# Yelp/nrtsearch

Hardware: AMD Instinct MI355X
Metric: queries/sec, 10M-doc 5-term BM25 top-1000 (higher is better)
Workload: dtype f32

## Files before the change

include/nrtgpu_dev.h:

```cpp
#ifndef NRTGPU_DEV_H
#define NRTGPU_DEV_H
#include "nrtgpu.h"
#ifdef __cplusplus
extern "C" {
#endif
int  nrtgpu_bench_closed_loop(nrtgpu_ctx* ctx, const nrtgpu_seg* const* segs, const int32_t* doc_bases, int32_t n_segs,
                              const nrtgpu_bm25_query* queries, int32_t n_queries, int32_t clients, int32_t duration_ms,
                              double* out4);
int  nrtgpu_debug_hold_coalescers(nrtgpu_ctx* ctx, int32_t hold);
int  nrtgpu_debug_coalescer_pending(nrtgpu_ctx* ctx, int32_t which);
int  nrtgpu_debug_dist_inject(nrtgpu_ctx* ctx, int32_t step, int32_t failed_query);
int64_t nrtgpu_debug_live_segments(nrtgpu_ctx* ctx);
int  nrtgpu_debug_spec_counters(nrtgpu_ctx* ctx, int64_t* out3);
int  nrtgpu_debug_term_lookup(const nrtgpu_seg* seg, int32_t field_id, int64_t term_hash, int32_t* kind, int32_t* shift, int64_t* bytes);
int  nrtgpu_debug_knn_bounds(int32_t sim, int32_t dim, double q_norm2, double q_l1, float q_absmax, double nv_max, double nv_min,
                             float rows_absmax, float score_boost, double m, double s, double* out10);
int  nrtgpu_debug_knn_unpack(const float* scores, const int32_t* docs, const uint32_t* counts, int32_t k_stride, int32_t n_queries,
                             int32_t k_pass, const int32_t* ks, const float* boosts, nrtgpu_topdocs* out);

#define NRTGPU_FLAG_PROFILE (7 << 8)
int  nrtgpu_get_scan_profile(nrtgpu_ctx* ctx, double* out16);
int  nrtgpu_get_maxscore_profile(nrtgpu_ctx* ctx, double* out16);
int  nrtgpu_debug_maxscore_meetings(nrtgpu_ctx* ctx, int64_t* out4);
int  nrtgpu_debug_maxscore_meeting_guesses(nrtgpu_ctx* ctx, int64_t* out1);
int  nrtgpu_debug_wave_kth(const uint64_t* keys, int32_t n, int32_t r, uint64_t* out);
int64_t nrtgpu_debug_walk_rows(nrtgpu_ctx* ctx, const nrtgpu_seg* const* segs, const int32_t* doc_bases, int32_t n_segs,
                               const nrtgpu_bm25_query* queries, int32_t n_queries, int32_t* out_begin, int32_t* out_n,
                               uint64_t* out_rows, int64_t cap_rows);
int  nrtgpu_debug_walk_value(float weight, const uint32_t* freq, const uint32_t* norm, int32_t n, const float* table256, int32_t fx_scale,
                             uint32_t fx_shift, uint64_t* out);
int64_t nrtgpu_get_maxscore_item_walls(nrtgpu_ctx* ctx, uint64_t* out, int64_t cap_slots, int64_t* n_items);

#ifdef __cplusplus
}
#endif
#endif
```

nrtsearch_amd/_lib.py:

```python
from __future__ import annotations

import ctypes as C
import os

_HERE = os.path.dirname(os.path.abspath(__file__))
LIB_PATH = os.environ.get("NRTGPU_LIB_PATH") or os.path.join(_HERE, "libnrtgpu.so")

NRTGPU_OK = 0
NRTGPU_ERR_INVALID_ARG = -1
NRTGPU_ERR_HIP = -2
NRTGPU_ERR_OOM = -3
NRTGPU_ERR_UNSUPPORTED = -4
NRTGPU_ERR_STATE = -5
NRTGPU_ERR_TIMEOUT = -6
NRTGPU_MAX_K = 1024
NRTGPU_MAX_TERMS = 32
NRTGPU_TILE_DOCS = 1024
NRTGPU_FLAG_NO_PREFETCH = 1
NRTGPU_FLAG_NO_FIXED_POINT = 2
NRTGPU_FLAG_NO_MASK_VARIANT = 4
NRTGPU_FLAG_NO_LIVE_FOLD = 8
NRTGPU_FLAG_NO_PRUNE = 16
NRTGPU_FLAG_PACKED_POSTINGS = 32
NRTGPU_FLAG_BLOCKING_WAIT = 64
NRTGPU_FLAG_NO_VECTOR_SKETCH = 128
NRTGPU_FLAG_PROFILE = 7 << 8
NRTGPU_MAX_MASKS = 8
NRTGPU_MAX_FUNCTIONS = 8
NRTGPU_MAX_GROUPS = 8
NRTGPU_GROUPS_SUM_OF_MAX = 0
NRTGPU_GROUPS_MAX_OF_SUM = 1
NRTGPU_MAX_KNN_LISTS = 8
NRTGPU_DOCVALUES_INT32 = 0
NRTGPU_DOCVALUES_FLOAT32 = 1
NRTGPU_MAX_TERM_BUCKETS = 65536

ABI_SYMBOLS = [
    "nrtgpu_version", "nrtgpu_last_error", "nrtgpu_create", "nrtgpu_destroy",
    "nrtgpu_segment_begin", "nrtgpu_segment_add_field_norms", "nrtgpu_segment_add_terms",
    "nrtgpu_segment_add_vectors", "nrtgpu_segment_seal", "nrtgpu_segment_set_live_docs",
    "nrtgpu_segment_set_mask", "nrtgpu_segment_release", "nrtgpu_segment_device_bytes",
    "nrtgpu_search_bm25", "nrtgpu_search_bm25_batch", "nrtgpu_search_bm25_batch_device",
    "nrtgpu_search_bm25_batch_device_epoch", "nrtgpu_exchange_open", "nrtgpu_exchange_close",
    "nrtgpu_search_bm25_coalesced", "nrtgpu_set_coalescing", "nrtgpu_query_supported",
    "nrtgpu_merge_topk_device", "nrtgpu_knn_exact", "nrtgpu_knn_exact_coalesced", "nrtgpu_knn_search", "nrtgpu_knn_search_requests", "nrtgpu_knn_search_coalesced", "nrtgpu_rescore_vectors", "nrtgpu_search_hybrid_batch",
    "nrtgpu_int_to_byte4", "nrtgpu_byte4_to_int", "nrtgpu_bm25_idf", "nrtgpu_bm25_avgdl",
    "nrtgpu_bm25_norm_cache", "nrtgpu_slices", "nrtgpu_plan_item_counts", "nrtgpu_fixed_point_scale", "nrtgpu_get_stats", "nrtgpu_reset_stats",
    "nrtgpu_set_slicing",
    "nrtgpu_blend", "nrtgpu_dist_unique_id", "nrtgpu_dist_init", "nrtgpu_dist_search_bm25_batch", "nrtgpu_dist_allgather_merge", "nrtgpu_segment_fork",
    "nrtgpu_search_bm25_batch_device_begin", "nrtgpu_pending_wait", "nrtgpu_set_thread_deadline_ns", "nrtgpu_monotonic_ns", "nrtgpu_last_diagnostics", "nrtgpu_dist_close", "nrtgpu_dist_owned_range", "nrtgpu_dist_search_bm25_batch_mode", "nrtgpu_dist_exchange_merge", "nrtgpu_dist_exchange_merge_checked", "nrtgpu_search_bm25_shard_device_begin", "nrtgpu_note_shard_speculation", "nrtgpu_dist_knn_exact", "nrtgpu_dist_search_hybrid_batch",
    "nrtgpu_knn_exact_relation", "nrtgpu_set_speculation", "nrtgpu_set_shard_share", "nrtgpu_set_thread_slices",
    "nrtgpu_segment_add_byte_vectors", "nrtgpu_knn_exact_bytes", "nrtgpu_knn_search_bytes", "nrtgpu_byte_vector_score",
    "nrtgpu_knn_search_bytes_requests", "nrtgpu_knn_search_bytes_coalesced", "nrtgpu_knn_exact_bytes_coalesced",
    "nrtgpu_rescore_byte_vectors", "nrtgpu_search_hybrid_bytes_batch", "nrtgpu_set_knn_gather",
    "nrtgpu_search_function_score_batch", "nrtgpu_function_score_supported", "nrtgpu_function_score_value",
    "nrtgpu_search_multi_match_batch", "nrtgpu_multi_match_supported", "nrtgpu_multi_match_value",
    "nrtgpu_search_function_score_multi_match_batch", "nrtgpu_function_score_multi_match_supported", "nrtgpu_function_score_multi_match_value",
    "nrtgpu_search_text_knn_batch", "nrtgpu_text_knn_supported", "nrtgpu_text_knn_value", "nrtgpu_text_knn_exact",
    "nrtgpu_segment_add_doc_values", "nrtgpu_search_sorted_batch", "nrtgpu_sorted_supported", "nrtgpu_sort_value_code",
    "nrtgpu_count_terms_batch", "nrtgpu_count_terms_supported",
]
DEV_SYMBOLS = [
    "nrtgpu_bench_closed_loop", "nrtgpu_debug_hold_coalescers", "nrtgpu_debug_coalescer_pending", "nrtgpu_debug_live_segments",
    "nrtgpu_debug_spec_counters", "nrtgpu_get_scan_profile", "nrtgpu_get_maxscore_profile", "nrtgpu_get_maxscore_item_walls",
    "nrtgpu_debug_dist_inject", "nrtgpu_debug_term_lookup", "nrtgpu_debug_knn_bounds", "nrtgpu_debug_knn_unpack",
    "nrtgpu_debug_maxscore_meetings", "nrtgpu_debug_wave_kth", "nrtgpu_debug_walk_rows", "nrtgpu_debug_walk_value",
    "nrtgpu_debug_maxscore_meeting_guesses",
]
DEV_LIB_PATH = os.path.join(_HERE, "libnrtgpu_dev.so")


class Config(C.Structure):
    _fields_ = [("device_id", C.c_int32), ("max_batch", C.c_int32), ("target_items", C.c_int32),
                ("collect_timing", C.c_int32), ("flags", C.c_int32), ("host_threads", C.c_int32),
                ("lookup_budget_pct", C.c_int32), ("reserved", C.c_int32)]


class Term(C.Structure):
    _fields_ = [("field_id", C.c_int32), ("cache_slot", C.c_int32), ("term_hash", C.c_int64),
                ("weight", C.c_float), ("occur", C.c_int32)]


class Bm25Query(C.Structure):
    _fields_ = [("n_terms", C.c_int32), ("terms", C.POINTER(Term)), ("n_caches", C.c_int32),
                ("norm_cache", C.POINTER(C.c_float)), ("k", C.c_int32), ("total_hits_threshold", C.c_int32),
                ("has_after", C.c_int32), ("after_doc", C.c_int32), ("after_score", C.c_float),
                ("min_should_match", C.c_int32), ("min_competitive_score", C.c_float), ("filter_mask", C.c_int32),
                ("must_not_mask", C.c_int32), ("disjunction_max", C.c_int32),
                ("n_more_filters", C.c_int32), ("more_filters", C.POINTER(C.c_int32)),
                ("n_more_must_not", C.c_int32), ("more_must_not", C.POINTER(C.c_int32)),
                ("tie_breaker", C.c_float), ("reserved", C.c_int32)]


class ScoreFunction(C.Structure):
    _fields_ = [("filter_mask", C.c_int32), ("weight", C.c_float)]


class FunctionScore(C.Structure):
    _fields_ = [("n_functions", C.c_int32), ("functions", C.POINTER(ScoreFunction)), ("score_mode", C.c_int32),
                ("boost_mode", C.c_int32), ("min_score", C.c_float), ("min_excluded", C.c_int32)]


class ClauseGroups(C.Structure):
    _fields_ = [("shape", C.c_int32), ("n_groups", C.c_int32), ("group_of_term", C.POINTER(C.c_int32)),
                ("group_min_should_match", C.POINTER(C.c_int32)), ("tie_breaker", C.c_float), ("group_occur", C.c_int32)]


class DocScores(C.Structure):
    _fields_ = [("docs", C.POINTER(C.c_int32)), ("scores", C.POINTER(C.c_float)), ("n", C.c_int32), ("boost", C.c_float)]


class KnnClauses(C.Structure):
    _fields_ = [("lists", C.POINTER(DocScores)), ("n_lists", C.c_int32), ("text_nested", C.c_int32)]


class TopDocs(C.Structure):
    _fields_ = [("n_hits", C.c_int32), ("capacity", C.c_int32), ("docs", C.POINTER(C.c_int32)),
                ("scores", C.POINTER(C.c_float)), ("total_hits", C.c_int64),
                ("total_hits_is_lower_bound", C.c_int32)]


class FieldSort(C.Structure):
    _fields_ = [("field_id", C.c_int32), ("reverse", C.c_int32), ("missing_bits", C.c_uint32), ("has_after", C.c_int32),
                ("after_doc", C.c_int32), ("after_bits", C.c_uint32)]


class FieldDocs(C.Structure):
    _fields_ = [("n_hits", C.c_int32), ("capacity", C.c_int32), ("docs", C.POINTER(C.c_int32)),
                ("value_bits", C.POINTER(C.c_uint32)), ("total_hits", C.c_int64),
                ("total_hits_is_lower_bound", C.c_int32)]


class TermsCount(C.Structure):
    _fields_ = [("field_id", C.c_int32), ("max_buckets", C.c_int32)]


class TermCounts(C.Structure):
    _fields_ = [("n_buckets", C.c_int32), ("capacity", C.c_int32), ("value_bits", C.POINTER(C.c_uint32)), ("counts", C.POINTER(C.c_int32)),
                ("total_hits", C.c_int64), ("hits_with_value", C.c_int64), ("overflowed", C.c_int32), ("reserved", C.c_int32)]


class Diagnostics(C.Structure):
    _fields_ = [("total_ms", C.c_double), ("plan_ms", C.c_double), ("queue_ms", C.c_double), ("device_ms", C.c_double),
                ("postings", C.c_int64), ("queries", C.c_int32), ("items_maxscore", C.c_int32), ("items_scan", C.c_int32),
                ("reserved", C.c_int32)]


class Stats(C.Structure):
    _fields_ = [("batches", C.c_int64), ("queries", C.c_int64), ("scan_launches", C.c_int64),
                ("scan_ms", C.c_double), ("scan_postings", C.c_int64), ("scan_items", C.c_int64),
# ... 65 lines not shown
    L.nrtgpu_exchange_close.restype = None
    L.nrtgpu_merge_topk_device.argtypes = [vp, i32, i32, i32, vp, vp, vp, vp, vp, C.POINTER(TopDocs)]
    L.nrtgpu_knn_exact.argtypes = [vp, vp, vp, i32, i32, i32, vp, i32, i32, i32, f32, C.POINTER(TopDocs)]
    L.nrtgpu_knn_exact_coalesced.argtypes = [vp, vp, vp, i32, i32, i32, vp, i32, i32, f32, C.POINTER(TopDocs)]
    L.nrtgpu_knn_exact_coalesced.restype = i32
    L.nrtgpu_knn_search.argtypes = [vp, vp, vp, i32, i32, i32, vp, i32, i32, i32, f32, i32, f32, C.POINTER(TopDocs)]
    L.nrtgpu_knn_search_requests.argtypes = [vp, vp, vp, i32, i32, i32, vp, i32, i32, vp, vp, vp, vp, C.POINTER(TopDocs)]
    L.nrtgpu_knn_search_coalesced.argtypes = [vp, vp, vp, i32, i32, i32, vp, i32, i32, f32, i32, f32, C.POINTER(TopDocs)]
    L.nrtgpu_knn_search_coalesced.restype = i32
    L.nrtgpu_segment_add_byte_vectors.argtypes = [vp, i32, i32, i32, vp, vp]
    L.nrtgpu_knn_exact_bytes.argtypes = [vp, vp, vp, i32, i32, i32, vp, i32, i32, i32, f32, C.POINTER(TopDocs)]
    L.nrtgpu_knn_search_bytes.argtypes = [vp, vp, vp, i32, i32, i32, vp, i32, i32, i32, f32, i32, f32, C.POINTER(TopDocs)]
    L.nrtgpu_knn_search_bytes_requests.argtypes = [vp, vp, vp, i32, i32, i32, vp, i32, i32, vp, vp, vp, vp, C.POINTER(TopDocs)]
    L.nrtgpu_knn_search_bytes_coalesced.argtypes = [vp, vp, vp, i32, i32, i32, vp, i32, i32, f32, i32, f32, C.POINTER(TopDocs)]
    L.nrtgpu_knn_search_bytes_coalesced.restype = i32
    L.nrtgpu_knn_exact_bytes_coalesced.argtypes = [vp, vp, vp, i32, i32, i32, vp, i32, i32, f32, C.POINTER(TopDocs)]
    L.nrtgpu_knn_exact_bytes_coalesced.restype = i32
    L.nrtgpu_byte_vector_score.argtypes = [i32, i32, i32, i32, i32, vp]
    L.nrtgpu_set_knn_gather.argtypes = [vp, i32]
    L.nrtgpu_search_function_score_batch.argtypes = [vp, vp, vp, i32, C.POINTER(Bm25Query), C.POINTER(FunctionScore), i32, C.POINTER(TopDocs)]
    L.nrtgpu_function_score_supported.argtypes = [vp, vp, i32, C.POINTER(Bm25Query), C.POINTER(FunctionScore)]
    L.nrtgpu_function_score_value.argtypes = [C.POINTER(FunctionScore), C.c_uint32, f32, vp, vp]
    L.nrtgpu_search_multi_match_batch.argtypes = [vp, vp, vp, i32, C.POINTER(Bm25Query), C.POINTER(ClauseGroups), i32, C.POINTER(TopDocs)]
    L.nrtgpu_multi_match_supported.argtypes = [vp, vp, i32, C.POINTER(Bm25Query), C.POINTER(ClauseGroups)]
    L.nrtgpu_multi_match_value.argtypes = [C.POINTER(ClauseGroups), i32, vp, i32, vp, C.c_uint32, vp, vp]
    L.nrtgpu_search_function_score_multi_match_batch.argtypes = [vp, vp, vp, i32, C.POINTER(Bm25Query), C.POINTER(ClauseGroups), C.POINTER(FunctionScore), i32,
                                                                 C.POINTER(TopDocs)]
    L.nrtgpu_function_score_multi_match_supported.argtypes = [vp, vp, i32, C.POINTER(Bm25Query), C.POINTER(ClauseGroups), C.POINTER(FunctionScore)]
    L.nrtgpu_function_score_multi_match_value.argtypes = [C.POINTER(ClauseGroups), i32, vp, i32, vp, C.c_uint32, C.POINTER(FunctionScore), C.c_uint32, vp, vp]
    L.nrtgpu_search_text_knn_batch.argtypes = [vp, vp, vp, i32, C.POINTER(Bm25Query), C.POINTER(KnnClauses), i32, C.POINTER(TopDocs)]
    L.nrtgpu_text_knn_supported.argtypes = [vp, vp, i32, C.POINTER(Bm25Query), C.POINTER(KnnClauses)]
    L.nrtgpu_text_knn_value.argtypes = [i32, i32, C.c_uint64, i32, C.c_double, vp]
    L.nrtgpu_text_knn_exact.argtypes = [C.POINTER(Bm25Query), C.POINTER(KnnClauses), i32]
    L.nrtgpu_segment_add_doc_values.argtypes = [vp, i32, i32, i32, vp, vp]
    L.nrtgpu_search_sorted_batch.argtypes = [vp, vp, vp, i32, C.POINTER(Bm25Query), C.POINTER(FieldSort), i32, C.POINTER(FieldDocs)]
    L.nrtgpu_sorted_supported.argtypes = [vp, vp, i32, C.POINTER(Bm25Query), C.POINTER(FieldSort)]
    L.nrtgpu_sort_value_code.argtypes = [i32, i32, C.c_uint32, vp]
    L.nrtgpu_count_terms_batch.argtypes = [vp, vp, vp, i32, C.POINTER(Bm25Query), C.POINTER(TermsCount), i32, C.POINTER(TermCounts)]
    L.nrtgpu_count_terms_supported.argtypes = [vp, vp, i32, C.POINTER(Bm25Query), C.POINTER(TermsCount)]
    L.nrtgpu_rescore_vectors.argtypes = [vp, vp, vp, i32, i32, i32, vp, i32, f32, vp, vp, i32, C.c_double, C.c_double, i32,
                                         C.POINTER(TopDocs)]
    L.nrtgpu_search_hybrid_batch.argtypes = [vp, vp, vp, i32, C.POINTER(Bm25Query), i32, i32, i32, vp, i32, f32,
                                             C.c_double, C.c_double, i32, C.POINTER(TopDocs)]
    L.nrtgpu_rescore_byte_vectors.argtypes = L.nrtgpu_rescore_vectors.argtypes
    L.nrtgpu_search_hybrid_bytes_batch.argtypes = L.nrtgpu_search_hybrid_batch.argtypes
    L.nrtgpu_int_to_byte4.argtypes = [i32]
    L.nrtgpu_byte4_to_int.argtypes = [i32]
    L.nrtgpu_bm25_idf.argtypes = [i64, i64]
    L.nrtgpu_bm25_idf.restype = f32
    L.nrtgpu_bm25_avgdl.argtypes = [i64, i64]
    L.nrtgpu_bm25_avgdl.restype = f32
    L.nrtgpu_bm25_norm_cache.argtypes = [f32, f32, f32, vp]
    L.nrtgpu_bm25_norm_cache.restype = None
    L.nrtgpu_plan_item_counts.argtypes = [i32, vp, i32, vp]
    L.nrtgpu_fixed_point_scale.argtypes = [f32, vp, i32, vp]
    L.nrtgpu_slices.argtypes = [i32, vp, vp, vp, i32, i32, i32, vp, vp]
    L.nrtgpu_get_stats.argtypes = [vp, C.POINTER(Stats)]
    L.nrtgpu_reset_stats.argtypes = [vp]
    L.nrtgpu_set_thread_slices.argtypes = [vp, i32]
    L.nrtgpu_set_speculation.argtypes = [vp, C.c_float]
    L.nrtgpu_set_speculation.restype = C.c_int
    L.nrtgpu_set_shard_share.argtypes = [vp, C.c_int64, C.c_int64]
    L.nrtgpu_set_shard_share.restype = C.c_int
    L.nrtgpu_knn_exact_relation.argtypes = [vp, vp, vp, C.c_int32, C.c_int32, C.c_int32, C.c_int32]
    L.nrtgpu_reset_stats.restype = None
    if hasattr(L, "nrtgpu_debug_hold_coalescers"):
        L.nrtgpu_debug_hold_coalescers.argtypes = [vp, C.c_int32]
        L.nrtgpu_debug_live_segments.argtypes = [vp]
        L.nrtgpu_debug_live_segments.restype = C.c_int64
        L.nrtgpu_debug_spec_counters.argtypes = [vp, vp]
        L.nrtgpu_debug_spec_counters.restype = C.c_int
        L.nrtgpu_get_maxscore_item_walls.argtypes = [vp, vp, C.c_int64, C.POINTER(C.c_int64)]
        L.nrtgpu_get_maxscore_item_walls.restype = C.c_int64
        L.nrtgpu_debug_coalescer_pending.argtypes = [vp, C.c_int32]
        L.nrtgpu_debug_dist_inject.argtypes = [vp, C.c_int32, C.c_int32]
        L.nrtgpu_get_scan_profile.argtypes = [vp, vp]
        L.nrtgpu_get_maxscore_profile.argtypes = [vp, vp]
        L.nrtgpu_debug_term_lookup.argtypes = [vp, i32, i64, C.POINTER(i32), C.POINTER(i32), C.POINTER(i64)]
    if hasattr(L, "nrtgpu_debug_maxscore_meetings"):
        L.nrtgpu_debug_maxscore_meetings.argtypes = [vp, vp]
        L.nrtgpu_debug_wave_kth.argtypes = [vp, i32, i32, vp]
    if hasattr(L, "nrtgpu_debug_maxscore_meeting_guesses"):
        L.nrtgpu_debug_maxscore_meeting_guesses.argtypes = [vp, vp]
    if hasattr(L, "nrtgpu_debug_walk_rows"):
        L.nrtgpu_debug_walk_rows.argtypes = [vp, vp, vp, i32, vp, i32, vp, vp, vp, i64]
        L.nrtgpu_debug_walk_rows.restype = C.c_int64
        L.nrtgpu_debug_walk_value.argtypes = [f32, vp, vp, i32, vp, i32, C.c_uint32, vp]
    if hasattr(L, "nrtgpu_debug_knn_bounds"):
        L.nrtgpu_debug_knn_bounds.argtypes = [i32, i32, C.c_double, C.c_double, f32, C.c_double, C.c_double, f32, f32, C.c_double, C.c_double, vp]
    if hasattr(L, "nrtgpu_debug_knn_unpack"):
        L.nrtgpu_debug_knn_unpack.argtypes = [vp, vp, vp, i32, i32, i32, vp, vp, C.POINTER(TopDocs)]
    L.nrtgpu_set_slicing.argtypes = [vp, i32, i32, i32]
    L.nrtgpu_blend.argtypes = [i32, vp, vp, vp, vp, i32, i32, i32, i32, C.POINTER(TopDocs)]
    L.nrtgpu_dist_unique_id.argtypes = [vp]
    L.nrtgpu_dist_init.argtypes = [vp, i32, i32, vp]
    L.nrtgpu_dist_search_bm25_batch.argtypes = [vp, vp, vp, i32, C.POINTER(Bm25Query), i32, C.POINTER(TopDocs)]
    L.nrtgpu_dist_allgather_merge.argtypes = [vp, i32, i32, vp, vp, vp, vp, vp, C.POINTER(TopDocs)]
    L.nrtgpu_segment_fork.argtypes = [vp, vp, i32, C.POINTER(vp)]
    L.nrtgpu_search_bm25_batch_device_begin.argtypes = [vp, vp, vp, i32, C.POINTER(Bm25Query), i32, i32, vp, vp, vp, C.c_int64, vp]
    L.nrtgpu_pending_wait.argtypes = [vp]
    L.nrtgpu_set_thread_deadline_ns.argtypes = [C.c_int64]
    L.nrtgpu_set_thread_deadline_ns.restype = None
    L.nrtgpu_monotonic_ns.argtypes = []
    L.nrtgpu_monotonic_ns.restype = C.c_int64
    L.nrtgpu_last_diagnostics.argtypes = [vp]
    L.nrtgpu_dist_owned_range.argtypes = [vp, i32, i32, vp, vp]
    L.nrtgpu_dist_search_bm25_batch_mode.argtypes = [vp, vp, vp, i32, C.POINTER(Bm25Query), i32, i32, C.POINTER(TopDocs)]
    L.nrtgpu_dist_exchange_merge.argtypes = [vp, i32, i32, vp, vp, vp, vp, vp, i32, C.POINTER(TopDocs)]
    L.nrtgpu_dist_exchange_merge_checked.argtypes = [vp, i32, i32, vp, vp, vp, vp, vp, vp, i32, C.POINTER(TopDocs), vp, vp]
    L.nrtgpu_search_bm25_shard_device_begin.argtypes = [vp, vp, vp, i32, C.POINTER(Bm25Query), i32, i32, vp, vp, vp, i32, vp, vp]
    L.nrtgpu_note_shard_speculation.argtypes = [vp, vp, i32, i32, i32]
    L.nrtgpu_dist_knn_exact.argtypes = [vp, vp, vp, i32, i32, i32, vp, i32, i32, i32, C.c_float, i32, C.POINTER(TopDocs)]
    L.nrtgpu_dist_search_hybrid_batch.argtypes = [vp, vp, vp, i32, C.POINTER(Bm25Query), i32, i32, i32, vp, i32, C.c_float, C.c_double, C.c_double,
                                                  i32, i32, C.POINTER(TopDocs)]
    L.nrtgpu_dist_close.argtypes = [vp]
    L.nrtgpu_dist_close.restype = None
    return L


def check(rc: int) -> None:
    if rc != NRTGPU_OK:
        raise NrtGpuError(rc, load().nrtgpu_last_error().decode("utf-8", "replace"))
```

nrtsearch_amd/api.py:

```python
from __future__ import annotations

import ctypes as C
import dataclasses
import os
import threading
from typing import Dict, List, Optional, Sequence, Tuple, Union

import numpy as np

from . import _lib
from ._lib import NrtGpuError

INT_MAX = 2**31 - 1
TOTAL_HITS_THRESHOLD = 1000


EXCHANGE_ALLGATHER, EXCHANGE_ALLTOALL = 0, 1
EXCHANGE_NO_SPECULATION = 0x100


@dataclasses.dataclass(frozen=True)
class TermQuery:
    field: int
    term: int
# ... 260 lines not shown
    def idf(self, doc_freq: int, doc_count: int) -> np.float32:
        return np.float32(_lib.load().nrtgpu_bm25_idf(int(doc_count), int(doc_freq)))

    def avgdl(self, cs: CollectionStatistics) -> np.float32:
        return np.float32(_lib.load().nrtgpu_bm25_avgdl(int(cs.sum_total_term_freq), int(cs.doc_count)))

    def norm_cache(self, cs: CollectionStatistics) -> np.ndarray:
        out = np.zeros(256, dtype=np.float32)
        _lib.load().nrtgpu_bm25_norm_cache(C.c_float(float(self.avgdl(cs))), C.c_float(self.k1), C.c_float(self.b),
                                          out.ctypes.data)
        return out

    def scorer(self, boost: float, cs: CollectionStatistics, doc_freq: int) -> Tuple[np.float32, np.ndarray]:
        idf = self.idf(doc_freq, cs.doc_count)
        return np.float32(np.float32(boost) * idf), self.norm_cache(cs)


class GpuContext:
    def __init__(self, device_id: int = 0, max_batch: int = 1024, target_items: int = 0,
                 collect_timing: bool = False, flags: int = 0, host_threads: int = 0, lookup_budget_pct: int = 0):
        L = _lib.load()
        if os.environ.get("NRTGPU_PACKED_POSTINGS", "") not in ("", "0"):
            flags |= _lib.NRTGPU_FLAG_PACKED_POSTINGS
        self.flags = flags
        if lookup_budget_pct == 0 and os.environ.get("NRTGPU_TEST_LOOKUP_BUDGET_PCT"):
            lookup_budget_pct = int(os.environ["NRTGPU_TEST_LOOKUP_BUDGET_PCT"])
        cfg = _lib.Config(device_id, max_batch, target_items, int(collect_timing), flags, host_threads, int(lookup_budget_pct), 0)
        h = C.c_void_p()
        _lib.check(L.nrtgpu_create(C.byref(cfg), C.byref(h)))
        self._h = h
        self.max_batch = max_batch

    def set_slicing(self, slice_max_docs: int = 250_000, slice_max_segments: int = 5, virtual_shards: int = 1) -> None:
        _lib.check(_lib.load().nrtgpu_set_slicing(self._h, int(slice_max_docs), int(slice_max_segments), int(virtual_shards)))

    @staticmethod
    def dist_unique_id() -> bytes:
        buf = C.create_string_buffer(128)
        _lib.check(_lib.load().nrtgpu_dist_unique_id(buf))
        return bytes(buf.raw)

    def dist_init(self, world: int, rank: int, unique_id: bytes) -> None:
        _lib.check(_lib.load().nrtgpu_dist_init(self._h, int(world), int(rank), C.c_char_p(unique_id)))

    def dist_close(self) -> None:
        _lib.load().nrtgpu_dist_close(self._h)

    def exchange_open(self, shm_name: str, world: int, rank: int) -> None:
        _lib.check(_lib.load().nrtgpu_exchange_open(self._h, shm_name.encode(), int(world), int(rank)))

    def exchange_close(self) -> None:
        _lib.load().nrtgpu_exchange_close(self._h)

    def stats(self) -> dict:
        st = _lib.Stats()
        _lib.check(_lib.load().nrtgpu_get_stats(self._h, C.byref(st)))
        return {n: getattr(st, n) for n, _ in _lib.Stats._fields_}

    def scan_profile(self) -> dict:
        out = np.zeros(16, dtype=np.float64)
        _lib.check(_lib.load().nrtgpu_get_scan_profile(self._h, out.ctypes.data))
        names = ["prologue_cycles", "rendezvous_wait_cycles", "rendezvous_cycles", "walk_cycles", "epilogue_cycles",
                 "rendezvous", "compactions", "subtiles", "rz_select_cycles", "sparse_subtiles", "rz_keep_cycles",
                 "rz_publish_append_cycles", "candidate_subtiles", "maybe_subtiles", "last_wave_finish_cycles",
                 "first_wave_finish_cycles"]
        return dict(zip(names, out.tolist()))

    def maxscore_profile(self) -> dict:
        out = np.zeros(16, dtype=np.float64)
        _lib.check(_lib.load().nrtgpu_get_maxscore_profile(self._h, out.ctypes.data))
        names = ["windows", "compactions", "chunks", "postings_streamed", "postings_surviving", "docs_evaluated", "lookups",
                 "candidates", "prologue_cycles", "item_cycles", "waves_meeting_cycles", "waves_idle_cycles", "waves_part_prologue_cycles",
                 "waves_walk_cycles", "last_wave_out_cycles", "epilogue_cycles"]
        return dict(zip(names, out.tolist()))

    def maxscore_meetings(self) -> dict:
        out = np.zeros(4, dtype=np.int64)
        _lib.check(_lib.load().nrtgpu_debug_maxscore_meetings(self._h, out.ctypes.data))
        res = dict(zip(["meetings", "overflow_meetings", "compactions", "wave_estimates"], (int(x) for x in out)))
        g = np.zeros(1, dtype=np.int64)
        _lib.check(_lib.load().nrtgpu_debug_maxscore_meeting_guesses(self._h, g.ctypes.data))
        res["meeting_guesses"] = int(g[0])
        return res

    @staticmethod
    def set_thread_deadline(seconds_from_now: Optional[float]) -> None:
        L = _lib.load()
        L.nrtgpu_set_thread_deadline_ns(0 if seconds_from_now is None else int(L.nrtgpu_monotonic_ns() + seconds_from_now * 1e9))

    @staticmethod
    def last_diagnostics() -> dict:
        d = _lib.Diagnostics()
        _lib.check(_lib.load().nrtgpu_last_diagnostics(C.byref(d)))
        return {n: getattr(d, n) for n, _ in _lib.Diagnostics._fields_ if n != "reserved"}

    def reset_stats(self) -> None:
        _lib.load().nrtgpu_reset_stats(self._h)

    def maxscore_item_walls(self):
        L = _lib.load()
        n_items = C.c_int64(0)
        n = int(L.nrtgpu_get_maxscore_item_walls(self._h, None, 0, C.byref(n_items)))
        out = np.zeros((max(n, 0), 8), dtype=np.uint64)
        if n > 0:
            L.nrtgpu_get_maxscore_item_walls(self._h, out.ctypes.data, n, C.byref(n_items))
        return out, int(n_items.value)

    @staticmethod
    def set_thread_slices(slice_of_leaf: Optional[Sequence[int]]) -> None:
        if slice_of_leaf is None:
            _lib.check(_lib.load().nrtgpu_set_thread_slices(None, 0))
        else:
            a = np.ascontiguousarray(slice_of_leaf, dtype=np.int32)
            _lib.check(_lib.load().nrtgpu_set_thread_slices(a.ctypes.data, len(a)))

    def set_speculation(self, margin: float) -> None:
        _lib.check(_lib.load().nrtgpu_set_speculation(self._h, C.c_float(float(margin))))

    def set_knn_gather(self, max_accept_permille: int) -> None:
        _lib.check(_lib.load().nrtgpu_set_knn_gather(self._h, int(max_accept_permille)))

    def set_shard_share(self, shard_docs: int, index_docs: int) -> None:
        _lib.check(_lib.load().nrtgpu_set_shard_share(self._h, int(shard_docs), int(index_docs)))

    def spec_counters(self) -> dict:
        st = self.stats()
        return {"queries": int(st["spec_queries"]), "reruns": int(st["spec_reruns"]), "switched_off": bool(st["spec_disabled"]),
                "scattered": bool(st["spec_scattered"])}

    def debug_live_segments(self) -> int:
        return int(_lib.load().nrtgpu_debug_live_segments(self._h))

    def debug_hold_coalescers(self, hold: bool) -> None:
        _lib.check(_lib.load().nrtgpu_debug_hold_coalescers(self._h, 1 if hold else 0))

    def debug_coalescer_pending(self, which: int) -> int:
        return int(_lib.load().nrtgpu_debug_coalescer_pending(self._h, int(which)))

    def debug_dist_inject(self, step: int = -1, failed_query: int = -1) -> None:
        _lib.check(_lib.load().nrtgpu_debug_dist_inject(self._h, int(step), int(failed_query)))

    def close(self) -> None:
        if getattr(self, "_h", None):
            _lib.load().nrtgpu_destroy(self._h)
            self._h = None

    def __del__(self):
        try:
            self.close()
        except Exception:
            pass


class GpuSegment:

    def __init__(self, ctx: GpuContext, max_doc: int, doc_base: int = 0):
        self.ctx, self.max_doc, self.doc_base = ctx, int(max_doc), int(doc_base)
        h = C.c_void_p()
        _lib.check(_lib.load().nrtgpu_segment_begin(ctx._h, self.max_doc, 0, C.byref(h)))
        self._h = h

    @classmethod
    def from_data(cls, ctx: GpuContext, seg, field: int = 0, omit_norms: bool = False,
                  omit_freqs: bool = False) -> "GpuSegment":
        g = cls(ctx, seg.max_doc, seg.doc_base)
        g.add_field_norms(field, None if omit_norms else seg.norms)
# ... 852 lines not shown
```

nrtsearch_amd/csrc/devtools.cpp:

```cpp
#include "runtime_internal.h"
#include "../../include/nrtgpu_dev.h"

extern "C" int nrtgpu_bench_closed_loop(nrtgpu_ctx* ctx, const nrtgpu_seg* const* segs, const int32_t* doc_bases,
                                        int32_t n_segs, const nrtgpu_bm25_query* queries, int32_t n_queries,
                                        int32_t clients, int32_t duration_ms, double* out4) {
  if (!ctx || !queries || !out4 || n_queries <= 0 || clients <= 0 || duration_ms <= 0)
    return fail(NRTGPU_ERR_INVALID_ARG, "bad closed-loop arguments");
  std::vector<std::vector<float>> lat((size_t)clients);
  std::vector<int> rcs((size_t)clients, 0);
  std::vector<std::string> errs((size_t)clients);
  const auto t_begin = std::chrono::steady_clock::now();
  const auto t_stop = t_begin + std::chrono::milliseconds(duration_ms);
  auto client = [&](int c) {
    int32_t kmax = 1;
    for (int i = 0; i < n_queries; ++i) kmax = std::max(kmax, queries[i].k);
    std::vector<int32_t> docs((size_t)kmax);
    std::vector<float> scores((size_t)kmax);
    size_t i = (size_t)c * 7919u;
    for (;;) {
      const auto t0 = std::chrono::steady_clock::now();
      if (t0 >= t_stop) break;
      nrtgpu_topdocs o{};
      o.capacity = kmax;
      o.docs = docs.data();
      o.scores = scores.data();
      const int rc = nrtgpu_search_bm25_coalesced(ctx, segs, doc_bases, n_segs, &queries[i % (size_t)n_queries], &o);
      if (rc != 0) {
        rcs[(size_t)c] = rc;
        errs[(size_t)c] = g_last_error;
        break;
      }
      lat[(size_t)c].push_back(std::chrono::duration<float, std::milli>(std::chrono::steady_clock::now() - t0).count());
      ++i;
    }
  };
  std::vector<std::thread> pool;
  for (int c = 0; c < clients; ++c) pool.emplace_back(client, c);
  for (auto& t : pool) t.join();
  const double secs = std::chrono::duration<double>(std::chrono::steady_clock::now() - t_begin).count();
  for (int c = 0; c < clients; ++c)
    if (rcs[(size_t)c] != 0) return fail(rcs[(size_t)c], "client %d: %s", c, errs[(size_t)c].c_str());
  std::vector<float> all;
  for (auto& v : lat) all.insert(all.end(), v.begin(), v.end());
  std::sort(all.begin(), all.end());
  out4[0] = (double)all.size();
  out4[1] = secs;
  out4[2] = all.empty() ? 0.0 : all[all.size() / 2];
  out4[3] = all.empty() ? 0.0 : all[(size_t)((double)all.size() * 0.99)];
  return NRTGPU_OK;
}


extern "C" int nrtgpu_debug_knn_bounds(int32_t sim, int32_t dim, double q_norm2, double q_l1, float q_absmax, double nv_max, double nv_min,
                                       float rows_absmax, float score_boost, double m, double s, double* out10) {
  if (!out10 || sim < 0 || sim > 3 || dim <= 0 || (dim & 15)) return fail(NRTGPU_ERR_INVALID_ARG, "bad knn_bounds arguments");
  float q_scale = 1.0f, rows_scale = 1.0f;
  const bool q_ok = hostmath::knn_sketch_scale(q_absmax, &q_scale), rows_ok = hostmath::knn_sketch_scale(rows_absmax, &rows_scale);
  const double e_rel = (double)hostmath::knn_e_rel(), b = (double)score_boost;
  const float e32 = hostmath::knn_bound32(sim, dim, q_norm2, nv_max, b);
  const float e16 = hostmath::knn_bound16(sim, dim, q_norm2, q_l1, 1.0 / (double)q_scale, nv_max, nv_min, 1.0 / (double)rows_scale, b);
  out10[0] = (double)e32;
  out10[1] = (double)e16;
  out10[2] = knn_result_upper(sim, m, (double)e32, e_rel, b);
  out10[3] = knn_result_upper(sim, m, (double)e16, e_rel, b);
  out10[4] = knn_estimate_lower(sim, s, (double)e32, e_rel, b);
  out10[5] = knn_estimate_lower(sim, s, (double)e16, e_rel, b);
  out10[6] = (double)q_scale;
  out10[7] = (double)rows_scale;
  out10[8] = q_ok ? 1.0 : 0.0;
  out10[9] = rows_ok ? 1.0 : 0.0;
  return NRTGPU_OK;
}

extern "C" int nrtgpu_debug_knn_unpack(const float* scores, const int32_t* docs, const uint32_t* counts, int32_t k_stride, int32_t n_queries,
                                       int32_t k_pass, const int32_t* ks, const float* boosts, nrtgpu_topdocs* out) {
  if (!scores || !docs || !counts || !out || n_queries <= 0 || k_pass <= 0 || k_stride < k_pass) return fail(NRTGPU_ERR_INVALID_ARG, "bad knn_unpack arguments");
  std::vector<uint64_t> keys((size_t)n_queries * (size_t)k_stride, 0ull);
  for (size_t i = 0; i < keys.size(); ++i)
    if ((uint32_t)(i % (size_t)k_stride) < counts[i / (size_t)k_stride]) keys[i] = pack_key(scores[i], (uint32_t)docs[i]);
  const KnnUniform one{k_pass, 0, 1.0f, 0.0f};
  std::vector<int32_t> k_of((size_t)n_queries, k_pass);
  std::vector<float> boost_of((size_t)n_queries, 1.0f);
  const KnnAsk each{ks ? ks : k_of.data(), boosts ? boosts : boost_of.data(), nullptr, nullptr, 1};
  knn_unpack_topdocs(keys.data(), counts, (uint32_t)k_stride, n_queries, false, 0, true, ks || boosts ? each : one.ask(), out);
  return NRTGPU_OK;
}

extern "C" int nrtgpu_debug_knn_query_stats(const float* queries, int32_t n_queries, int32_t dim, float* norm2, float* max_abs, double* l1,
                                            float* ref_norm2) {
  if (!queries || !norm2 || !max_abs || !l1 || !ref_norm2 || n_queries <= 0 || dim <= 0) return fail(NRTGPU_ERR_INVALID_ARG, "bad knn_query_stats arguments");
  knn_query_stats(queries, n_queries, dim, norm2, max_abs, l1);
  for (int32_t q = 0; q < n_queries; ++q) ref_norm2[q] = float_qnorm2(queries + (size_t)q * dim, dim);
  return NRTGPU_OK;
}

extern "C" int nrtgpu_debug_maxscore_meetings(nrtgpu_ctx* ctx, int64_t* out4) {
  if (!ctx || !out4) return fail(NRTGPU_ERR_INVALID_ARG, "NULL argument");
  std::lock_guard<std::mutex> lk(ctx->stats_mu);
  for (int i = 0; i < 4; ++i) out4[i] = ctx->ms_meetings[i];
  return NRTGPU_OK;
}

extern "C" int nrtgpu_debug_maxscore_meeting_guesses(nrtgpu_ctx* ctx, int64_t* out1) {
  if (!ctx || !out1) return fail(NRTGPU_ERR_INVALID_ARG, "NULL argument");
  std::lock_guard<std::mutex> lk(ctx->stats_mu);
  *out1 = ctx->ms_meetings[4];
  return NRTGPU_OK;
}

extern "C" int nrtgpu_debug_wave_kth(const uint64_t* keys, int32_t n, int32_t r, uint64_t* out) {
  if (!keys || !out || n < 1 || n > kMsCandCap || r < 1 || r > n) return fail(NRTGPU_ERR_INVALID_ARG, "bad wave_kth arguments (1 <= r <= n <= %d)", kMsCandCap);
  uint64_t* d = nullptr;
  if (hipMalloc((void**)&d, ((size_t)n + 1) * sizeof(uint64_t)) != hipSuccess) return fail(NRTGPU_ERR_OOM, "hipMalloc");
  hipError_t e = hipMemcpy(d, keys, (size_t)n * sizeof(uint64_t), hipMemcpyHostToDevice);
  if (e == hipSuccess) {
    launch_debug_wave_kth(nullptr, d, (uint32_t)n, (uint32_t)r, d + n);
    e = hipGetLastError();
  }
  if (e == hipSuccess) e = hipMemcpy(out, d + n, sizeof(uint64_t), hipMemcpyDeviceToHost);
  (void)hipFree(d);
  if (e != hipSuccess) return fail(NRTGPU_ERR_HIP, "wave_kth: %s", hipGetErrorString(e));
  return NRTGPU_OK;
}

extern "C" int64_t nrtgpu_debug_walk_rows(nrtgpu_ctx* ctx, const nrtgpu_seg* const* segs, const int32_t* doc_bases, int32_t n_segs,
                                          const nrtgpu_bm25_query* queries, int32_t n_queries, int32_t* out_begin, int32_t* out_n,
                                          uint64_t* out_rows, int64_t cap_rows) {
  if (!ctx || !segs || !queries || !out_begin || !out_n || (!out_rows && cap_rows > 0)) return -(int64_t)fail(NRTGPU_ERR_INVALID_ARG, "NULL argument");
  if (n_queries <= 0 || n_segs <= 0 || cap_rows < 0) return -(int64_t)fail(NRTGPU_ERR_INVALID_ARG, "n_queries and n_segs must be > 0");
  if (hipSetDevice(ctx->device) != hipSuccess) return -(int64_t)fail(NRTGPU_ERR_HIP, "hipSetDevice");
  for (int si = 0; si < n_segs; ++si)
    if (!segs[si]) return -(int64_t)fail(NRTGPU_ERR_INVALID_ARG, "segment %d is NULL", si);
  SegReadLocks content(segs, n_segs);
  HostPlan hp;
  if (int rc = build_plan(ctx, segs, doc_bases, n_segs, queries, n_queries, hp, 1)) return -(int64_t)rc;
  const size_t n_pairs = (size_t)n_queries * (size_t)n_segs;
  for (size_t i = 0; i < n_pairs; ++i) out_begin[i] = -1, out_n[i] = 0;
  if (hp.n_dterms == 0) return 0;
  Carver c;
  const size_t o_qx = c.take(sizeof(DExpandHead) + hp.qexpand.size() * sizeof(DQExpand)) + sizeof(DExpandHead), o_qt = c.take(hp.qterms.size() * sizeof(DQTerm));
  const size_t o_qsb = c.take(hp.qs_begin.size() * 4), o_caches = c.take(hp.caches.size() * sizeof(float));
  const size_t o_queries = c.take(hp.queries.size() * sizeof(DQuery)), o_up = c.off;
  const size_t o_terms = c.take((size_t)hp.n_dterms * sizeof(DTerm)), o_rows = c.take((size_t)hp.n_dterms * sizeof(DWalkRow));
  std::vector<char> hb(c.off, 0);
  memcpy(hb.data() + o_qx, hp.qexpand.data(), hp.qexpand.size() * sizeof(DQExpand));
  if (!hp.qterms.empty()) memcpy(hb.data() + o_qt, hp.qterms.data(), hp.qterms.size() * sizeof(DQTerm));
  memcpy(hb.data() + o_qsb, hp.qs_begin.data(), hp.qs_begin.size() * 4);
  if (!hp.caches.empty()) memcpy(hb.data() + o_caches, hp.caches.data(), hp.caches.size() * sizeof(float));
  memcpy(hb.data() + o_queries, hp.queries.data(), hp.queries.size() * sizeof(DQuery));
  char* db = nullptr;
  if (hipMalloc((void**)&db, c.off) != hipSuccess) return -(int64_t)fail(NRTGPU_ERR_OOM, "hipMalloc");
  DExpandHead xh{};
  xh.caches = (const float*)(db + o_caches);
  xh.queries = (const DQuery*)(db + o_queries);
  xh.rows = (DWalkRow*)(db + o_rows);
  memcpy(hb.data() + o_qx - sizeof(DExpandHead), &xh, sizeof(xh));
  hipError_t e = hipMemcpy(db, hb.data(), o_up, hipMemcpyHostToDevice);
  if (e == hipSuccess) e = hipMemset(db + o_up, 0, c.off - o_up);
  if (e == hipSuccess) {
    launch_expand_terms(nullptr, (const DQExpand*)(db + o_qx), (const DQTerm*)(db + o_qt), (const uint32_t*)(db + o_qsb), (uint32_t)n_queries,
                        hp.n_leaves, (DTerm*)(db + o_terms));
    e = hipGetLastError();
  }
  if (e == hipSuccess) e = hipMemcpy(hb.data() + o_rows, db + o_rows, (size_t)hp.n_dterms * sizeof(DWalkRow), hipMemcpyDeviceToHost);
  (void)hipFree(db);
  if (e != hipSuccess) return -(int64_t)fail(NRTGPU_ERR_HIP, "walk_rows: %s", hipGetErrorString(e));
  static_assert(sizeof(DWalkRow) == 80, "ten words per row");
  if (out_rows) memcpy(out_rows, hb.data() + o_rows, (size_t)std::min<int64_t>(cap_rows, (int64_t)hp.n_dterms) * sizeof(DWalkRow));
  std::vector<uint32_t> begins;
  for (size_t i = 0; i < n_pairs; ++i)
    if (hp.qs_begin[i] != 0xFFFFFFFFu) begins.push_back(hp.qs_begin[i]);
  std::sort(begins.begin(), begins.end());
  for (size_t i = 0; i < n_pairs; ++i) {
    const uint32_t b = hp.qs_begin[i];
    if (b == 0xFFFFFFFFu || hp.qexpand[i / (size_t)n_segs].by_weight == 0u) continue;
    auto nx = std::upper_bound(begins.begin(), begins.end(), b);
    out_begin[i] = (int32_t)b;
    out_n[i] = (int32_t)((nx == begins.end() ? hp.n_dterms : *nx) - b);
  }
  return (int64_t)hp.n_dterms;
}

extern "C" int nrtgpu_debug_walk_value(float weight, const uint32_t* freq, const uint32_t* norm, int32_t n, const float* table256, int32_t fx_scale,
                                       uint32_t fx_shift, uint64_t* out) {
  if (!freq || !norm || !table256 || !out || n < 1 || fx_shift > 31u) return fail(NRTGPU_ERR_INVALID_ARG, "bad walk_value arguments");
// ... 17 lines not shown
```

nrtsearch_amd/csrc/maxscore.hip:

```cpp
#include <hip/hip_runtime.h>
#include <stdint.h>

#include <type_traits>

#include "bm25_common.hiph"

namespace nrtgpu {

constexpr int kMsWinWords = kMsWinDocs / 32;
constexpr int kSl = kMsSlots;
typedef uint32_t u32x2 __attribute__((ext_vector_type(2)));
typedef const NRT_GLOBAL u32x2* gvec2_ptr;

struct alignas(16) WClause {
  uint64_t docids, fnorm;
  uint64_t begin;
  uint32_t count, pad0;
  float    weight;
  int32_t  fx_scale;
  uint32_t flags;
  uint32_t pad;
  uint64_t u_after;
  uint64_t look;
  uint64_t cells, start;
// ... 150 lines not shown
      const uint64_t pb = exchange_bound(*xch, query, q2_hi != 0u ? (uint64_t)q2_hi << 32 : 0ull, tid);
      if (tid == 0 && pb > s.theta) {
        s.theta = pb;
        s.thr = acc_threshold<true>(pb, fx_E);
        atomicMax(theta_g, (unsigned long long)pb);
      }
    }
  } else {
    if (r != 0u && cnt0 > r) guess = topk_kth_union<kMsThreads>(s.cand, cnt0, r, &s.sc, [](auto&&) {}, 0u);
    if (tid == 0) s.cnt = cnt0;
  }
  if (tid == 0 && s.spec_z16 != 0u) {
    if (guess > s.theta) {
      s.theta = guess;
      s.thr = acc_threshold<true>(guess, fx_E);
      atomicMax(theta_g, (unsigned long long)guess);
      atomicMax(s.spec_slot, (unsigned long long)guess);
      s.n_est += 0x10000u;
    }
    const uint32_t ws = s.wins_started;
    s.spec_at = ws >= s.q_wins ? 0u : max(ws * s.spec_grow16 / 16u, ws + (uint32_t)kMsWaves);
  }
  __syncthreads();
  if (tid == 0) s.rz_flag = 0;
  __syncthreads();
}

__device__ __forceinline__ bool ms_meet(MsSmem& s, uint32_t k, int fx_E, unsigned long long* theta_g, const DExchange* xch = nullptr,
                                        uint32_t query = 0) {
  __syncthreads();
  if (!__hip_atomic_load(&s.rz_flag, __ATOMIC_RELAXED, __HIP_MEMORY_SCOPE_WORKGROUP)) return false;
  ms_compact((__attribute__((address_space(3))) MsSmem*)&s, k, fx_E, theta_g, xch, query);
  return true;
}

__device__ __noinline__ void ms_estimate(__attribute__((address_space(3))) MsSmem* sp, uint32_t k, int fx_E,
                                         unsigned long long* theta_g, const DExchange* xch) {
  MsSmem& s = *(MsSmem*)sp;
  const uint32_t lane = threadIdx.x & 63u;
  const uint32_t ws = (uint32_t)__builtin_amdgcn_readfirstlane((int)__hip_atomic_load(&s.wins_started, __ATOMIC_RELAXED, __HIP_MEMORY_SCOPE_WORKGROUP));
  const uint32_t at = (uint32_t)__builtin_amdgcn_readfirstlane((int)__hip_atomic_load(&s.spec_at, __ATOMIC_RELAXED, __HIP_MEMORY_SCOPE_WORKGROUP));
  const uint32_t n = (uint32_t)__builtin_amdgcn_readfirstlane((int)__hip_atomic_load(&s.cnt, __ATOMIC_RELAXED, __HIP_MEMORY_SCOPE_WORKGROUP));
  if (at != 0u && ws >= at && n <= (uint32_t)kMsCandCap) {
    const bool exchanging = xch && xch->world > 1u;
    uint32_t r = 0;
    if (s.spec_z16 != 0u && !exchanging && __hip_atomic_load(&s.prune_on, __ATOMIC_RELAXED, __HIP_MEMORY_SCOPE_WORKGROUP) != 0u) {
      const float m = (float)k * fminf(1.0f, (float)ws / (float)max(s.q_wins, 1u));
      const float rr = m + (float)s.spec_z16 * (1.0f / 16.0f) * sqrtf(m) + 2.0f;
      r = rr < (float)k ? (uint32_t)rr : 0u;
    }
    uint64_t guess = 0;
    if (r != 0u && n > r) guess = topk_kth_wave(s.cand, n, r, &s.sc);
    if (lane == 0u) {
      if (guess > s.theta) {
        __hip_atomic_store(&s.theta, guess, __ATOMIC_RELAXED, __HIP_MEMORY_SCOPE_WORKGROUP);
        __hip_atomic_store(&s.thr, acc_threshold<true>(guess, fx_E), __ATOMIC_RELAXED, __HIP_MEMORY_SCOPE_WORKGROUP);
        atomicMax(theta_g, (unsigned long long)guess);
        atomicMax(s.spec_slot, (unsigned long long)guess);
      }
      s.spec_at = ws >= s.q_wins ? 0u : max(ws * s.spec_grow16 / 16u, ws + (uint32_t)kMsWaves);
      s.n_est += 1u;
    }
  }
  wave_lds_phase();
  if (lane == 0u) __hip_atomic_store(&s.spec_busy, 0u, __ATOMIC_RELEASE, __HIP_MEMORY_SCOPE_WORKGROUP);
}

__device__ __forceinline__ bool ms_reserve(MsSmem& s, uint32_t lane, uint32_t mine, uint32_t& pos) {
  const uint32_t incl = scan64_dpp(mine);
  const uint32_t wave_total = (uint32_t)__builtin_amdgcn_readlane((int)incl, 63);
  uint32_t wbase = 0;
  if (lane == 0) {
    wbase = atomicAdd(&s.cnt, wave_total);
    if (wbase + wave_total > (uint32_t)kMsCandCap) {
      if (wbase <= (uint32_t)kMsCandCap) s.cnt_valid = wbase;
      __hip_atomic_store(&s.rz_flag, 1u, __ATOMIC_RELAXED, __HIP_MEMORY_SCOPE_WORKGROUP);
    }
  }
  wbase = (uint32_t)__builtin_amdgcn_readfirstlane((int)wbase);
  pos = wbase + incl - mine;
  return wbase + wave_total <= (uint32_t)kMsCandCap;
}

template <bool PROF, bool PACKED, int SHAPES>
__global__ __launch_bounds__(kMsThreads)
void bm25_maxscore_kernel(const MsArgs* __restrict__ launch) {
  constexpr bool TWO = SHAPES == 2;
  constexpr bool kMsHalfBody = kSl == 8;
  __shared__ MsSmem s;
  const uint32_t tid = threadIdx.x;
  const uint32_t wave = tid >> 6, lane = tid & 63u;
  for (uint32_t round = 0;; ++round) {
    const uint64_t wall_entry = PROF ? wall_clock64() : 0ull;
    const ms_args_ptr ap = ms_fresh(launch);
    const __attribute__((address_space(4))) DHelp& hp = ap->help;
    const DItem* const items = as_global(ap->items);
    const DPart* const parts = as_global(ap->parts);
    const DWalkRow* const rows = as_global(ap->rows);
  #ifdef NRTGPU_DEV
    const DTerm* const terms = as_global(ap->terms);
  #endif
    const DExchange* const xch = as_global(ap->xch);
    bool helper = false;
    uint32_t my_item = 0, out_slot = 0;
    {
      const uint32_t min_rem = hp.min_rem & 0xFFFFu;
      const bool greedy = ((hp.min_rem >> 16) & 1u) != 0u;
      for (int attempt = 0; attempt < 2; ++attempt) {
        if (tid == 0) {
          s.pick = 0ull;
          s.role[0] = __hip_atomic_load(hp.item_next, __ATOMIC_RELAXED, __HIP_MEMORY_SCOPE_AGENT);
          s.role[1] = __hip_atomic_load(hp.help_used, __ATOMIC_RELAXED, __HIP_MEMORY_SCOPE_AGENT);
          s.role[2] = 0u;
          s.role[3] = __hip_atomic_load(hp.help_off, __ATOMIC_RELAXED, __HIP_MEMORY_SCOPE_AGENT);
        }
        __syncthreads();
        const uint32_t q_next = s.role[0];
        const bool queue_empty = attempt == 1 || q_next >= hp.n_own;
        const bool slots_left = s.role[1] < hp.n_help;
        if (queue_empty && (!slots_left || s.role[3] != 0u)) return;
        const bool look = slots_left && (queue_empty || (hp.alpha16 != 0u && q_next >= hp.n_cus + hp.n_cus / 4u));
        if (look) {
          const uint64_t now = wall_clock64();
          float t_rem = 0.f;
          if (!queue_empty) {
            uint32_t mine = 0;
            for (uint32_t i = tid; i < hp.n_own; i += kMsThreads) {
              const uint64_t t0 = __hip_atomic_load(hp.item_t0 + i, __ATOMIC_RELAXED, __HIP_MEMORY_SCOPE_AGENT);
              if (t0 == 0ull) continue;
              mine += min(items[i].flags >> 8, (uint32_t)kMsWaves + __hip_atomic_load(hp.win_next + i, __ATOMIC_RELAXED, __HIP_MEMORY_SCOPE_AGENT));
            }
            mine = (uint32_t)__builtin_amdgcn_readlane((int)scan64_dpp(mine), 63);
            if (lane == 0 && mine != 0u) atomicAdd(&s.role[2], mine);
            __syncthreads();
            const uint32_t handed = s.role[2];
            const uint64_t ts = __hip_atomic_load(hp.t_start, __ATOMIC_RELAXED, __HIP_MEMORY_SCOPE_AGENT);
            t_rem = (handed == 0u || ts == 0ull || now <= ts) ? 3.0e38f
                    : (float)(now - ts) * (float)(hp.total_wins > handed ? hp.total_wins - handed : 0u) / (float)handed * ((float)hp.alpha16 * (1.0f / 16.0f));
          }
          for (uint32_t i = tid; i < hp.n_own; i += kMsThreads) {
            const uint32_t fl = items[i].flags;
            if ((fl & 3u) == kMsModeExact) continue;
            const uint32_t nw = fl >> 8;
            const uint32_t taken = (uint32_t)kMsWaves + __hip_atomic_load(hp.win_next + i, __ATOMIC_RELAXED, __HIP_MEMORY_SCOPE_AGENT);
            if (taken + min_rem > nw) continue;
            const uint64_t t0 = __hip_atomic_load(hp.item_t0 + i, __ATOMIC_RELAXED, __HIP_MEMORY_SCOPE_AGENT);
            if (t0 == 0ull || now <= t0) continue;
            const uint32_t hc = __hip_atomic_load(hp.help_cnt + i, __ATOMIC_RELAXED, __HIP_MEMORY_SCOPE_AGENT);
            const float left = (float)(now - t0) * (float)(nw - taken) / ((float)(taken - (uint32_t)kMsWaves + 1u) * (float)(1u + hc));
            if (!queue_empty && !(left > t_rem)) continue;
            uint32_t hsh = ((blockIdx.x + round * gridDim.x) * 0x9E3779B9u) ^ (i * 0x85EBCA6Bu) ^ (uint32_t)now;
            hsh ^= hsh >> 16; hsh *= 0x7FEB352Du; hsh ^= hsh >> 15; hsh *= 0x846CA68Bu; hsh ^= hsh >> 16;
            const float u = ((float)(hsh >> 8) + 0.5f) * (1.0f / 16777216.0f);
            const float key = greedy ? left : left / -__logf(u);
            atomicMax((unsigned long long*)&s.pick, ((unsigned long long)__float_as_uint(key) << 32) | (unsigned long long)(i + 1u));
          }
        }
        __syncthreads();
        if (tid == 0) {
          const uint64_t pick = s.pick;
          uint32_t r_item = 0xFFFFFFFFu, r_slot = 0xFFFFFFFFu;
          if ((uint32_t)pick != 0u) {
            const uint32_t slot = atomicAdd(hp.help_used, 1u);
            if (slot < hp.n_help) {
              r_slot = slot;
              r_item = (uint32_t)pick - 1u;
              atomicAdd(hp.help_cnt + r_item, 1u);
            }
          } else if (queue_empty && look) {
            __hip_atomic_store(hp.help_off, 1u, __ATOMIC_RELAXED, __HIP_MEMORY_SCOPE_AGENT);
          }
          if (r_slot == 0xFFFFFFFFu && !queue_empty) {
            const uint32_t it = atomicAdd(hp.item_next, 1u);
            if (it < hp.n_own) r_item = it;
          }
          s.role[0] = r_item;
          s.role[1] = r_slot;
        }
        __syncthreads();
        const uint32_t r_item = s.role[0], r_slot = s.role[1];
        __syncthreads();
        if (r_item != 0xFFFFFFFFu) {
          my_item = r_item;
          helper = r_slot != 0xFFFFFFFFu;
          out_slot = helper ? hp.slot_base + r_slot : r_item;
          break;
        }
        if (queue_empty) return;
      }
    }
    NRT_GLOBAL uint32_t* const win_next_g = (NRT_GLOBAL uint32_t*)(hp.win_next + my_item);
    uint32_t first_win = 0;
    if (helper && lane == 0) first_win = __hip_atomic_fetch_add(win_next_g, 1u, __ATOMIC_RELAXED, __HIP_MEMORY_SCOPE_AGENT);
    const DItem item = items[my_item];
    const DQuery q = as_global(ap->queries)[item.query];
    const uint32_t k = q.k;
    const int fx_E = item.fx_E;
    unsigned long long* const my_theta_g = as_global(ap->theta_g) + item.query;
    const bool multi_item = q.n_items > 1 || hp.n_help != 0u;
    const uint32_t mode = item.flags & 3u;
    const uint32_t win_tiles = (uint32_t)kMsWinTiles >> ((item.flags >> 2) & 3u);
    const uint32_t msm = SHAPES ? q.min_should_match : 0u;
    const bool use_max = SHAPES && q.combine_max != 0u;
    const uint32_t sec_mode = TWO ? q.sec_mode : kMsSecNone;
    const float tie_breaker = TWO ? q.tie_breaker : 0.0f;
    auto loosen = [&](uint64_t t) { return (TWO && sec_mode == kMsSecReqOpt) ? max(t - (t >> 21), (uint64_t)2) - (uint64_t)1 : t; };
    unsigned int* const my_prune_g = as_global(ap->q_prune) + item.query;
    const uint64_t after_key = q.has_after ? pack_key(q.after_score, (uint32_t)q.after_doc) : ~0ull;

    {
      const uint32_t n_lds = min(item.n_caches, (uint32_t)kLdsCaches) * 256u;
      const float* const caches = as_global(ap->caches);
      for (uint32_t i = tid; i < n_lds; i += kMsThreads) (&s.cache[0][0])[i] = caches[item.cache_off + i];
    }
    for (uint32_t i = tid; i < (uint32_t)kMsCandCap; i += kMsThreads) s.cand[i] = 0ull;
    if (tid == 0) {
      const uint64_t theta0 = __hip_atomic_load(my_theta_g, __ATOMIC_RELAXED, __HIP_MEMORY_SCOPE_AGENT);
      s.theta = theta0;
      s.thr = acc_threshold<true>(theta0, fx_E);
      s.cnt = 0;
      s.cnt_valid = 0;
      s.rz_flag = 0;
      s.spec_busy = 0;
      s.n_meet = s.n_over = s.n_est = 0;
      if (!helper) {
        const unsigned long long now0 = (unsigned long long)wall_clock64();
        __hip_atomic_store(hp.item_t0 + my_item, now0, __ATOMIC_RELAXED, __HIP_MEMORY_SCOPE_AGENT);
        if (my_item == 0u) __hip_atomic_store(hp.t_start, now0, __ATOMIC_RELAXED, __HIP_MEMORY_SCOPE_AGENT);
      }
      s.prune_on = mode == kMsModePrune ? 1u : 0u;
      const bool spec = hp.spec_g != nullptr && hp.spec_z16 != 0u;
      s.wins_started = 0;
      s.q_wins = spec ? as_global(ap->q_wins)[item.query] : 0u;
      s.spec_z16 = spec ? hp.spec_z16 : 0u;
      s.spec_slot = spec ? as_global(hp.spec_g) + item.query : nullptr;
      s.spec_at = spec ? max(hp.spec_sched & 255u, 1u) : 0u;
      s.spec_grow16 = max((hp.spec_sched >> 8) & 255u, 17u);
      s.spec_meet = (hp.spec_sched >> 16) & 7u;
      for (int i = 0; i < kSliceSlots; ++i) s.slot_hits[i] = s.slot_slice[i] = 0u;
      for (int i = 0; i < 16; ++i) s.prof[i] = 0;
    }
    const uint64_t t_item0 = PROF ? __builtin_readcyclecounter() : 0ull;
    const uint64_t wall0 = PROF ? wall_clock64() : 0ull;
    uint64_t tc_meet = 0, tc_part = 0, tc_walk = 0;
    __syncthreads();
    if (xch && tid < 64u) {
      const uint64_t pb = exchange_bound(*xch, item.query, 0ull, tid);
      if (tid == 0 && pb > s.theta) {
        s.theta = pb;
        s.thr = acc_threshold<true>(pb, fx_E);
      }
    }
    for (uint32_t slot = 0; slot < item.n_tabs; ++slot) {
      const float w = items[my_item].tab_weight[slot];
      const int scale = items[my_item].tab_scale[slot];
      const float* cache = &s.cache[items[my_item].tab_cache[slot]][0];
      for (uint32_t e = tid; e < (uint32_t)kTabEntries; e += kMsThreads)
        s.tab[slot][e] = e < (uint32_t)kTabNorms ? 0u : score_value<true>(bm25_score(w, (float)(int32_t)(e >> 7), cache[e & 127u]), scale);
    }
    __syncthreads();
  #if !defined(NRT_MS_PHASE_CLOCKS) && !defined(NRT_MS_COUNT_ROUNDS)
    if (PROF && tid == 0) s.prof[8] = __builtin_readcyclecounter() - t_item0;
  #endif

    uint32_t* const seen = &s.seen[wave][0];
    WClause* const wcl = &s.wc[wave][0];
    const uint32_t wcl_addr = lds_addr(wcl);
    uint32_t wave_hits = 0;
    uint32_t cur_slot = 0;
    uint64_t pc_post = 0, pc_surv = 0, pc_look = 0, pc_cand = 0, pc_chunks = 0, pc_wins = 0;
  #ifdef NRT_MS_PHASE_CLOCKS
    uint64_t ph[9] = {0, 0, 0, 0, 0, 0, 0, 0, 0}, ph_t = 0;
  #endif
  #ifdef NRT_MS_COUNT_ROUNDS
    uint64_t pc_dense = 0, pc_sparse = 0, pc_steps = 0, pc_tas = 0, pc_crounds = 0, pc_half = 0, pc_half_rounds = 0;
    uint64_t pc_cres = 0, pc_cinst = 0;
  #endif
    const uint32_t item_wins = item.flags >> 8;
    uint32_t sc_mul = 1u;
    if (ap->scatter != 0u && item_wins > 3u && item_wins < 65536u) {
      const uint32_t primes[4] = {2654435761u, 2246822519u, 3266489917u, 668265263u};
      uint32_t best = 0xFFFFFFFFu;
  #pragma unroll
      for (int i = 0; i < 4; ++i) {
        const uint32_t a = primes[i] % item_wins;
        const uint32_t x = a * 1000u, y = item_wins * 618u;
        const uint32_t dist = x > y ? x - y : y - x;
        if (a > 1u && dist < best) {
          best = dist;
          sc_mul = a;
        }
      }
    }
    auto window_of_take = [&](uint32_t h) -> uint32_t {
      return (sc_mul == 1u || h >= item_wins) ? h : (h * sc_mul) % item_wins;
    };
    uint32_t g = window_of_take(helper ? (uint32_t)kMsWaves + (uint32_t)__builtin_amdgcn_readfirstlane((int)first_win) : wave);
    uint32_t pi = 0;
    uint32_t win_base = 0;

    const bool parts_by_lane = item.n_parts <= 64u;
    uint32_t part_incl = 0;
    if (parts_by_lane) {
      uint32_t w = 0;
      if (lane < item.n_parts) {
        const u32x2 tr = *(gvec2_ptr)&parts[item.part_begin + lane].tile_begin;
        w = (tr[1] - (tr[0] & ~(win_tiles - 1u)) + win_tiles - 1u) / win_tiles;
      }
      part_incl = scan64_dpp(w);
    }

    for (;;) {
      DPart part;
      uint32_t part_wins = 0;
      if (parts_by_lane) {
        const uint64_t holds = __builtin_amdgcn_ballot_w64(lane < item.n_parts && g < part_incl);
        if (holds == 0ull) break;
        pi = (uint32_t)__builtin_ctzll(holds);
        part = parts[item.part_begin + pi];
        part_wins = (part.tile_end - (part.tile_begin & ~(win_tiles - 1u)) + win_tiles - 1u) / win_tiles;
        win_base = (uint32_t)__builtin_amdgcn_readlane((int)part_incl, (int)pi) - part_wins;
      } else {
        if (sc_mul != 1u) {
          pi = 0;
          win_base = 0;
        }
        for (;; ++pi) {
          if (pi >= item.n_parts) break;
          part = parts[item.part_begin + pi];
          part_wins = (part.tile_end - (part.tile_begin & ~(win_tiles - 1u)) + win_tiles - 1u) / win_tiles;
          if (g < win_base + part_wins) break;
          win_base += part_wins;
        }
      }
      if (pi >= item.n_parts) break;
      {
        const uint32_t p_slot = part.slice >> 24;
        if (p_slot != cur_slot && wave_hits != 0u) {
          if (lane == 0) atomicAdd(&s.slot_hits[cur_slot], wave_hits);
          wave_hits = 0;
        }
        cur_slot = p_slot;
        if (lane == 0) s.slot_slice[p_slot] = part.slice & 0xFFFFFFu;
      }
      const uint32_t n_terms = part.n_terms;
      uint64_t my_suf = 0, my_start = 0;
      gu32_ptr my_cells = nullptr;
      uint32_t my_shift = 0, my_flags = 0;
      const uint64_t t_part0 = PROF ? __builtin_readcyclecounter() : 0ull;
  #ifdef NRTGPU_DEV
      if (rows == nullptr) {
        const DTerm* const part_terms = terms + part.term_begin;
        uint64_t my_ub = 0;
// ... 37 lines not shown
        my_cells = (gu32_ptr)mt.cell_off;
        my_shift = mt.shift;
        my_start = mt.start;
        if (lane < n_terms) {
          WClause w;
          w.docids = (uint64_t)mt.docids;
          w.fnorm = (uint64_t)mt.fnorm;
          w.begin = 0;
          w.count = w.pad0 = 0;
          w.weight = mt.weight;
          w.fx_scale = mt.fx_scale;
          const DTermAux* const ax = mt.aux;
          const uint32_t look_kind = ax->look_kind;
          w.flags = ((mt.tab_slot & 0xFFFFu) < (uint32_t)kTabTerms ? (mt.tab_slot & 0xFFFFu) : 7u) | (TWO && (mt.tab_slot & kTabSlotRequired) ? 8u : 0u) |
                    (mt.fx_shift << 4) | (mt.cache_slot << 8) | ((mt.shift & 31u) << 16) | ((look_kind & 7u) << 24) | (((uint32_t)ax->look_shift & 31u) << 27);
          w.pad = 0;
          w.u_after = my_after;
          w.look = look_kind != kLookNone ? (uint64_t)ax->look : 0ull;
          w.cells = (uint64_t)mt.cell_off;
          w.start = mt.start;
          wcl[lane] = w;
          my_flags = w.flags;
        }
      } else
  #endif
      {
        static_assert(sizeof(DWalkRow) == sizeof(WClause) && sizeof(WClause) % 16 == 0, "a walk row is the image of a WClause");
        const gvec_ptr src = (gvec_ptr)(rows + part.term_begin);
        if (lane < n_terms * (uint32_t)(sizeof(WClause) / 16)) *(u32x4*)lds_ptr(wcl_addr + lane * 16u) = src[lane];
        wave_lds_phase();
        if (lane < n_terms) {
          const uint32_t rec = wcl_addr + lane * (uint32_t)sizeof(WClause);
          my_suf = *(const uint64_t*)lds_ptr(rec + 16u);
          my_flags = *(const uint32_t*)lds_ptr(rec + 40u);
          const u32x4 cs = *(const u32x4*)lds_ptr(rec + 64u);
          my_cells = (gu32_ptr)(((uint64_t)cs[1] << 32) | cs[0]);
          my_start = ((uint64_t)cs[3] << 32) | cs[2];
        }
        my_shift = (my_flags >> 16) & 31u;
      }
      const uint32_t req_mask = TWO ? (uint32_t)__builtin_amdgcn_ballot_w64(lane < n_terms && (my_flags & 8u) != 0u) : 0u;
      const uint32_t first_req = req_mask != 0u ? (uint32_t)__builtin_ctz(req_mask) : 0xFFu;
      if (PROF) tc_part += __builtin_readcyclecounter() - t_part0;

      for (;;) {
        const uint64_t t_win0 = PROF ? __builtin_readcyclecounter() : 0ull;
        const uint32_t ta = (part.tile_begin & ~(win_tiles - 1u)) + (g - win_base) * win_tiles;
        const uint32_t t0 = max(ta, part.tile_begin);
        const uint32_t t1 = min(ta + win_tiles, part.tile_end);
        const uint32_t doc_lo = t0 * (uint32_t)kTileDocs;
        const uint32_t doc_span = min(t1 * (uint32_t)kTileDocs, part.max_doc) - doc_lo;
        if (PROF) pc_wins += 1;
        {
          uint32_t est = 0;
          if (lane == 0) {
            const uint32_t ws = atomicAdd(&s.wins_started, 1u) + 1u, at = s.spec_at;
            if (at != 0u && ws >= at) {
              if ((s.spec_meet & 1u) != 0u) __hip_atomic_store(&s.rz_flag, 1u, __ATOMIC_RELAXED, __HIP_MEMORY_SCOPE_WORKGROUP);
              else est = atomicCAS(&s.spec_busy, 0u, 1u) == 0u ? 1u : 0u;
            }
          }
          if (__builtin_amdgcn_readfirstlane((int)est) != 0)
            ms_estimate((__attribute__((address_space(3))) MsSmem*)&s, k, fx_E, my_theta_g, xch);
        }
        uint32_t g_new = 0;
        if (lane == 0) g_new = (uint32_t)kMsWaves + __hip_atomic_fetch_add(win_next_g, 1u, __ATOMIC_RELAXED, __HIP_MEMORY_SCOPE_AGENT);
        uint64_t theta_other = 0, thr_other = 0;
        if (multi_item) {
          theta_other = __hip_atomic_load(my_theta_g, __ATOMIC_RELAXED, __HIP_MEMORY_SCOPE_AGENT);
          thr_other = acc_threshold<true>(theta_other, fx_E);
          if (mode == kMsModeCount && lane == 0 && __hip_atomic_load(my_prune_g, __ATOMIC_RELAXED, __HIP_MEMORY_SCOPE_AGENT) != 0u)
            __hip_atomic_store(&s.prune_on, 1u, __ATOMIC_RELAXED, __HIP_MEMORY_SCOPE_WORKGROUP);
        }
        uint32_t my_lo = 0, my_hi = 0;
        if (lane < n_terms) {
          my_lo = my_cells[t0 >> my_shift];
          my_hi = my_cells[((t1 - 1u) >> my_shift) + 1u];
        }
        if (n_terms > 1u) {
  #pragma unroll
          for (int j = 0; j < kMsWinWords / 64 / 4; ++j) *(u32x4*)&seen[(lane + 64u * (uint32_t)j) * 4u] = u32x4{0u, 0u, 0u, 0u};
        }
        uint32_t ng = 0;
        {
          const uint64_t thr_w = __hip_atomic_load(&s.prune_on, __ATOMIC_RELAXED, __HIP_MEMORY_SCOPE_WORKGROUP) ? loosen(max(s.thr, thr_other)) : 0ull;
          const uint64_t pb = my_start + my_lo, pe = my_start + my_hi;
          if (lane < n_terms) {
            if (my_suf >= thr_w && pe > pb && (!SHAPES || msm <= 1u || lane + msm <= n_terms) && (!TWO || lane <= first_req)) ng = (uint32_t)((pe - (pb & ~3ull) + (uint64_t)(kSl - 1)) / (uint64_t)kSl);
            *(u32x4*)&wcl[lane].begin = u32x4{(uint32_t)pb, (uint32_t)(pb >> 32), (uint32_t)(pe - pb), 0u};
          }
        }
        const uint32_t incl = scan32_dpp(ng);
        uint32_t pre[kMsMaxTerms];
  #pragma unroll
        for (int i = 0; i < kMsMaxTerms; ++i) pre[i] = (uint32_t)__builtin_amdgcn_readlane((int)incl, i);
        const uint32_t n_groups = pre[kMsMaxTerms - 1];
  #ifdef NRTGPU_DEV
        const bool half_on = (__builtin_amdgcn_readfirstlane((int)s.spec_meet) & 2) == 0;
  #else
        constexpr bool half_on = true;
  #endif

  #ifdef NRT_MS_PHASE_CLOCKS
        if (PROF) ph_t = t_win0;
  #endif
        NRT_PH_MARK(0);
        auto walk_units = [&](auto ns_c, auto half_c, const uint32_t v0) __attribute__((always_inline)) -> bool {
          constexpr int NS = decltype(ns_c)::value;
          constexpr bool HALF = decltype(half_c)::value;
          static_assert(!HALF || (NS == 4 && kSl == 8), "the half body: four of a unit's eight postings per lane");
          const uint32_t n_lanes = HALF ? 2u * (n_groups - v0) : min(n_groups - v0, 64u);
          const uint32_t v = HALF ? v0 + (lane >> 1) : v0 + lane;
          const bool act = HALF ? lane < n_lanes : v < n_groups;
          uint32_t c = 0, before = 0;
  #pragma unroll
          for (int i = 0; i < kMsMaxTerms - 1; ++i) {
            c += (v >= pre[i]) ? 1u : 0u;
            before = (v >= pre[i]) ? pre[i] : before;
          }
          const uint32_t c_first = (uint32_t)__builtin_amdgcn_readfirstlane((int)c);
          const uint64_t theta = max(s.theta, theta_other), thr = loosen(max(s.thr, thr_other));
          const bool pruning = __hip_atomic_load(&s.prune_on, __ATOMIC_RELAXED, __HIP_MEMORY_SCOPE_WORKGROUP) != 0u;
          const uint64_t thr_p = pruning ? thr : 0ull;
          if (readlane_u64(my_suf, c_first) < thr_p) return false;
          if (PROF) pc_chunks += 1;
          const uint32_t rec = wcl_addr + c * (uint32_t)sizeof(WClause);
          const u32x4 r0 = *(const u32x4*)lds_ptr(rec), r1 = *(const u32x4*)lds_ptr(rec + 16u), r2 = *(const u32x4*)lds_ptr(rec + 32u);
          const uint64_t u_after = *(const uint64_t*)lds_ptr(rec + 48u);
          const uint64_t col_d = ((uint64_t)r0[1] << 32) | r0[0], col_c = ((uint64_t)r0[3] << 32) | r0[2];
          const uint64_t p_begin = ((uint64_t)r1[1] << 32) | r1[0];
          const uint32_t flags = r2[2];
          const uint32_t q0 = (v - before) * (uint32_t)kSl + (HALF ? (lane & 1u) * 4u : 0u);
          const uint64_t mine0 = (p_begin & ~3ull) + (uint64_t)q0;
          uint32_t d[NS], cd[NS];
  #pragma unroll
          for (int j = 0; j < NS; ++j) d[j] = cd[j] = 0u;
          if (act) {
            const u32x4 d0 = __builtin_nontemporal_load((gvec_ptr)(col_d + mine0 * 4u));
            const u32x4 d1 = NS > 4 ? __builtin_nontemporal_load((gvec_ptr)(col_d + mine0 * 4u) + 1) : d0;
            if (PACKED) {
              const uint32_t sw = doc_lo & ~kPackDocMask;
  #pragma unroll
              for (int j = 0; j < 4; ++j) {
                d[j] = (d0[j] >> kPackCodeBits) | sw;
                cd[j] = (d0[j] & kPackCodeMask) << 2;
                if (NS > 4) {
                  d[(4 + j) % NS] = (d1[j] >> kPackCodeBits) | sw;
                  cd[(4 + j) % NS] = (d1[j] & kPackCodeMask) << 2;
                }
              }
            } else {
              const u32x4 c0 = __builtin_nontemporal_load((gvec_ptr)(col_c + mine0 * 4u));
              const u32x4 c1 = NS > 4 ? __builtin_nontemporal_load((gvec_ptr)(col_c + mine0 * 4u) + 1) : c0;
  #pragma unroll
              for (int j = 0; j < 4; ++j) {
                d[j] = d0[j];
                cd[j] = c0[j];
                if (NS > 4) {
                  d[(4 + j) % NS] = d1[j];
                  cd[(4 + j) % NS] = c1[j];
                }
              }
            }
          }
          NRT_PH_MARK(1);
          uint32_t vmask = 0;
          {
            const uint32_t rel = q0 - ((uint32_t)p_begin & 3u), cnt = act ? r1[2] : 0u;
  #pragma unroll
            for (int j = 0; j < NS; ++j)
              if (rel + (uint32_t)j < cnt && d[j] - doc_lo < doc_span) vmask |= 1u << j;
          }
          uint32_t val[NS];
          {
            const uint32_t tab = flags & 7u;
            const char* tb = (const char*)&s.tab[tab == 7u ? 0u : tab][0];
            uint32_t cor = 0;
  #pragma unroll
            for (int j = 0; j < NS; ++j) {
              val[j] = *(const uint32_t*)(tb + (cd[j] & 0x1FFCu));
              const uint32_t cn = ((vmask >> j) & 1u) ? cd[j] : 0u;
              cor = PACKED ? max(cor, cn) : (cor | cn);
            }
            const bool special = vmask != 0u && ((PACKED ? cor >= (kPackEscBase << 2) : (cor >> 31) != 0u) || tab == 7u);
            if (__any(special)) {
              const float w = __uint_as_float(r2[0]);
              const int fx_scale = (int)r2[1];
              const float* cache = &s.cache[(flags >> 8) & 255u][0];
  #pragma unroll
              for (int j = 0; j < NS; ++j) {
                uint32_t cj = cd[j];
                if (PACKED && cj >= (kPackEscBase << 2))
                  cj = ((vmask >> j) & 1u) ? packed_escape_word((gu32_ptr)col_c, (uint32_t)mine0 + (uint32_t)j, cj >> 2) : 0x80000100u;
                const bool esc = (cj >> 31) != 0u;
                const uint32_t f = esc ? ((cj >> 8) & 0x3FFFFFu) : ((cj >> 9) & 15u);
                const bool dead = esc ? ((cj >> 30) & 1u) != 0u : (cj >> 20) != 0u;
                const uint32_t nb = esc ? (cj & 255u) : ((cj >> 2) & 127u);
                if (((vmask >> j) & 1u) && (esc || tab == 7u))
                  val[j] = dead ? 0u : score_value<true>(bm25_score(w, (float)(int32_t)f, cache[nb]), fx_scale);
              }
            }
          }
          uint64_t run[NS];
          uint32_t alive = 0;
          {
            const uint32_t mult = 1u << ((flags >> 4) & 15u);
            uint32_t need_v = 1u;
            if (u_after < thr_p) {
              const uint64_t gap = use_max ? thr_p : thr_p - u_after;
              const uint64_t nv = (gap + (uint64_t)(mult - 1u)) >> ((flags >> 4) & 15u);
              need_v = nv > 0xFFFFFFFFull ? 0xFFFFFFFFu : max((uint32_t)nv, 1u);
            }
            uint32_t pass = 0;
  #pragma unroll
            for (int j = 0; j < NS; ++j) {
              run[j] = (uint64_t)val[j] * (uint64_t)mult;
              pass |= val[j] >= need_v ? (1u << j) : 0u;
            }
            alive = vmask & pass;
            if (need_v == 0xFFFFFFFFu) {
  #pragma unroll
              for (int j = 0; j < NS; ++j)
                if ((use_max ? max(run[j], u_after) : run[j] + u_after) < thr_p) alive &= ~(1u << j);
            }
          }
          uint64_t sec[TWO ? NS : 1];
          if (TWO) {
            if ((req_mask & ((1u << c) - 1u)) != 0u) alive = 0u;
            const bool mine_counts = sec_mode == kMsSecTieBreaker || (sec_mode == kMsSecReqOpt && ((req_mask >> c) & 1u) == 0u);
  #pragma unroll
            for (int j = 0; j < NS; ++j) sec[j] = mine_counts ? run[j] : 0ull;
          }
          if (PROF) {
            pc_post += (uint64_t)__popc(vmask);
            pc_surv += (uint64_t)__popc(alive);
          }
          NRT_PH_MARK(2);
          const uint32_t c_last = (uint32_t)__builtin_amdgcn_readlane((int)c, (int)(n_lanes - 1u));
          if (n_terms > 1u && __any(alive != 0u)) {
            for (uint32_t cc = c_first; cc <= c_last; ++cc) {
              const uint32_t am = c == cc ? alive : 0u;
              if (!__any(am != 0u)) continue;
  #ifdef NRT_MS_COUNT_ROUNDS
              if (PROF) pc_tas += 1;
  #endif
              uint32_t old[NS];
  #pragma unroll
              for (int j = 0; j < NS; ++j) {
                const bool a = (am >> j) & 1u;
                const uint32_t w = a ? ((d[j] - doc_lo) >> 5) : lane;
                old[j] = atomicOr(&seen[w], a ? (1u << (d[j] & 31u)) : 0u);
              }
  #pragma unroll
              for (int j = 0; j < NS; ++j)
                if (((am >> j) & 1u) && ((old[j] >> (d[j] & 31u)) & 1u)) alive &= ~(1u << j);
            }
          }
          NRT_PH_MARK(3);
          uint32_t ccnt = 0x11111111u;

          for (uint32_t j2 = c_first + 1u; j2 < n_terms; ++j2) {
            if (!__any(alive != 0u)) break;
            const uint64_t S_j = readlane_u64(my_suf, j2);
            uint32_t am = c < j2 ? alive : 0u;
            {
              const uint64_t short_of = S_j < thr_p ? (use_max ? thr_p : thr_p - S_j) : 0ull;
              uint32_t kill = 0;
  #pragma unroll
              for (int j = 0; j < NS; ++j) kill |= run[j] < short_of ? (1u << j) : 0u;
              if (SHAPES && msm > 1u) {
                const uint32_t left = n_terms - j2;
  #pragma unroll
                for (int j = 0; j < NS; ++j) kill |= ((ccnt >> (4 * j)) & 15u) + left < msm ? (1u << j) : 0u;
              }
              kill &= am;
              alive &= ~kill;
              am &= ~kill;
            }
            if (!__any(am != 0u)) continue;
            if (PROF) pc_look += (uint64_t)__popc(am);
            const WClause& w2 = wcl[j2];
            const uint64_t look2 = uniform_u64(w2.look);
            const uint32_t flags2 = (uint32_t)__builtin_amdgcn_readfirstlane((int)w2.flags);
            const uint32_t kind2 = (flags2 >> 24) & 7u;
            const uint64_t start2 = uniform_u64(w2.start);
            const gu32_ptr codes2 = (gu32_ptr)(uniform_u64(PACKED ? w2.docids : w2.fnorm) + start2 * 4u);
            uint32_t c2[NS];
            uint32_t pi2[NS];
            uint32_t present = 0;
  #ifdef NRT_MS_COUNT_ROUNDS
            if (PROF) { if (kind2 == kLookBits) pc_dense += 1; else pc_sparse += 1; }
  #endif
            if (kind2 == kLookBits) {
              const gvec2_ptr recs = (gvec2_ptr)look2;
              u32x2 r[NS];
  #pragma unroll
              for (int j = 0; j < NS; ++j) r[j] = recs[((am >> j) & 1u) ? (d[j] >> 5) : 0u];
              __builtin_amdgcn_sched_barrier(0);
              NRT_PH_MARK(4);
              uint32_t idx[NS];
  #pragma unroll
              for (int j = 0; j < NS; ++j) {
                const uint32_t bb = d[j] & 31u;
                const bool there = ((am >> j) & 1u) && ((r[j][0] >> bb) & 1u);
                idx[j] = there ? r[j][1] + (uint32_t)__popc(r[j][0] & ((1u << bb) - 1u)) : 0u;
                present |= (there ? 1u : 0u) << j;
              }
  #pragma unroll
              for (int j = 0; j < NS; ++j) c2[j] = codes2[idx[j]];
              __builtin_amdgcn_sched_barrier(0);
              NRT_PH_MARK(5);
  #pragma unroll
              for (int j = 0; j < NS; ++j) pi2[j] = (uint32_t)start2 + idx[j];
            } else {
              const gu32_ptr cells2 = (gu32_ptr)(kind2 == kLookCells ? look2 : uniform_u64(w2.cells));
              const gu32_ptr docs2 = (gu32_ptr)(uniform_u64(w2.docids) + start2 * 4u);
              const uint32_t cshift = kind2 == kLookCells ? (flags2 >> 27) & 31u : 10u + ((flags2 >> 16) & 31u);
              uint32_t a[NS], b[NS];
  #pragma unroll
              for (int j = 0; j < NS; ++j) {
                const uint32_t cell = ((am >> j) & 1u) ? (d[j] >> cshift) : 0u;
                a[j] = cells2[cell];
                b[j] = cells2[cell + 1u];
              }
              uint32_t open = 0;
  #pragma unroll
              for (int j = 0; j < NS; ++j) {
                if (!((am >> j) & 1u)) b[j] = a[j];
                open |= (a[j] < b[j] ? 1u : 0u) << j;
              }
              while (__any(open != 0u)) {
  #ifdef NRT_MS_COUNT_ROUNDS
                if (PROF) pc_steps += 1;
  #endif
                uint32_t mid[NS], vv[NS];
  #pragma unroll
                for (int j = 0; j < NS; ++j) {
                  mid[j] = (a[j] + b[j]) >> 1;
                  vv[j] = docs2[((open >> j) & 1u) ? mid[j] : 0u];
                }
  #pragma unroll
                for (int j = 0; j < NS; ++j)
                  if ((open >> j) & 1u) {
                    const uint32_t dv = PACKED ? vv[j] >> kPackCodeBits : vv[j], dd = PACKED ? d[j] & kPackDocMask : d[j];
                    if (dv < dd) a[j] = mid[j] + 1u;
                    else b[j] = mid[j];
                    if (dv == dd) {
                      a[j] = b[j] = mid[j];
                      present |= 1u << j;
                    }
                    if (!(a[j] < b[j])) open &= ~(1u << j);
                  }
              }
  #pragma unroll
              for (int j = 0; j < NS; ++j) {
                c2[j] = codes2[((present >> j) & 1u) ? a[j] : 0u];
                pi2[j] = (uint32_t)start2 + a[j];
              }
              NRT_PH_MARK(7);
            }
            if (__any(present != 0u)) {
              uint32_t v2[NS];
              if (PACKED) {
  #pragma unroll
                for (int j = 0; j < NS; ++j) c2[j] = (c2[j] & kPackCodeMask) << 2;
              }
              values_of_codes<PACKED, NS>(s, c2, present, flags2 & 7u, w2.weight, w2.fx_scale, (flags2 >> 8) & 255u, w2.fnorm, pi2, v2);
              const uint32_t mult2 = 1u << ((flags2 >> 4) & 15u);
              if (use_max) {
  #pragma unroll
                for (int j = 0; j < NS; ++j) run[j] = max(run[j], (uint64_t)(((present >> j) & 1u) ? v2[j] : 0u) * (uint64_t)mult2);
              } else if (TWO && sec_mode != kMsSecNone) {
                const bool counts = sec_mode == kMsSecReqOpt && (flags2 & 8u) == 0u;
  #pragma unroll
                for (int j = 0; j < NS; ++j) {
                  const uint64_t add = (uint64_t)(((present >> j) & 1u) ? v2[j] : 0u) * (uint64_t)mult2;
// ... 22 lines not shown
          for (int j = 0; j < NS; ++j)
            if (((alive >> j) & 1u) && run[j] >= thr) maybe |= 1u << j;
          {
            uint32_t pool = pruning ? maybe : alive;
            if (SHAPES && msm > 1u) {
  #pragma unroll
              for (int j = 0; j < NS; ++j)
                if (((ccnt >> (4 * j)) & 15u) < msm) pool &= ~(1u << j);
            }
            if (part.live_bits != nullptr && __any(pool != 0u)) {
              uint32_t lw[NS];
  #pragma unroll
              for (int j = 0; j < NS; ++j) lw[j] = ((const NRT_GLOBAL uint32_t*)part.live_bits)[((pool >> j) & 1u) ? (d[j] >> 5) : 0u];
  #pragma unroll
              for (int j = 0; j < NS; ++j)
                if (!((lw[j] >> (d[j] & 31u)) & 1u)) pool &= ~(1u << j);
            }
            maybe &= pool;
            uint32_t h = (uint32_t)__popc(pool);
            h = (uint32_t)__builtin_amdgcn_readlane((int)scan64_dpp(h), 63);
            if (mode == kMsModeCount && !pruning) {
              if (lane == 0 && h != 0u) {
                const uint32_t tot = atomicAdd(&s.slot_hits[cur_slot], h) + h;
                if (tot > q.gte_floor) {
                  __hip_atomic_store(&s.prune_on, 1u, __ATOMIC_RELAXED, __HIP_MEMORY_SCOPE_WORKGROUP);
                  if (multi_item) __hip_atomic_store(my_prune_g, 1u, __ATOMIC_RELAXED, __HIP_MEMORY_SCOPE_AGENT);
                }
              }
            } else {
              wave_hits += h;
            }
          }
          uint64_t theta_now = theta;
  #ifdef NRT_MS_COUNT_ROUNDS
          const uint64_t cres0 = pc_cres;
  #endif
          while (__any(maybe != 0u)) {
  #ifdef NRT_MS_COUNT_ROUNDS
            if (PROF) pc_crounds += 1;
  #endif
            const uint32_t low = maybe & (0u - maybe);
            uint64_t rsel = run[0], ssel = TWO ? sec[0] : 0ull;
            uint32_t dsel = d[0];
  #pragma unroll
            for (int j = 1; j < NS; ++j)
              if (low == (1u << j)) {
                rsel = run[j];
                dsel = d[j];
                if (TWO) ssel = sec[j];
              }
            float score = acc_score<true>(rsel, fx_E);
            if (TWO && sec_mode == kMsSecTieBreaker)
              score = (float)(ldexp((double)ssel, -fx_E) + ldexp((double)(rsel - ssel), -fx_E) * (double)tie_breaker);
            else if (TWO && sec_mode == kMsSecReqOpt)
              score = acc_score<true>(rsel - ssel, fx_E) + acc_score<true>(ssel, fx_E);
            const uint64_t key = pack_key(score, (uint32_t)(part.doc_base + (int32_t)dsel));
            const bool want = low != 0u && key > theta_now && key < after_key;
            uint32_t pos = 0;
            if (!__any(want)) {
              maybe &= ~low;
              continue;
            }
  #ifdef NRT_MS_COUNT_ROUNDS
            if (PROF) pc_cres += 1;
  #endif
            if (ms_reserve(s, lane, want ? 1u : 0u, pos)) {
              if (want) s.cand[pos] = key;
              if (PROF) pc_cand += want ? 1u : 0u;
              maybe &= ~low;
              continue;
            }
            const uint64_t t_m0 = PROF ? __builtin_readcyclecounter() : 0ull;
            (void)ms_meet(s, k, fx_E, my_theta_g, xch, item.query);
            if (PROF) tc_meet += __builtin_readcyclecounter() - t_m0;
            theta_now = max(theta_now, s.theta);
          }
  #ifdef NRT_MS_COUNT_ROUNDS
          if (PROF && pc_cres != cres0) pc_cinst += 1;
  #endif
          }
          NRT_PH_MARK(8);
          return true;
        };
        for (uint32_t v0 = 0; v0 < n_groups; v0 += 64u) {
          bool more;
          if (kMsHalfBody && n_groups - v0 <= 32u && half_on) {
  #ifdef NRT_MS_COUNT_ROUNDS
            const uint64_t chunks0 = pc_chunks, look0 = pc_dense + pc_sparse;
  #endif
            if constexpr (kMsHalfBody) more = walk_units(std::integral_constant<int, 4>{}, std::true_type{}, v0);
            else more = false;
  #ifdef NRT_MS_COUNT_ROUNDS
            if (PROF) {
              pc_half += pc_chunks - chunks0;
              pc_half_rounds += pc_dense + pc_sparse - look0;
            }
  #endif
          } else {
            more = walk_units(std::integral_constant<int, kSl>{}, std::false_type{}, v0);
          }
          if (!more) break;
          if (__hip_atomic_load(&s.rz_flag, __ATOMIC_RELAXED, __HIP_MEMORY_SCOPE_WORKGROUP)) {
            const uint64_t t_m0 = PROF ? __builtin_readcyclecounter() : 0ull;
            (void)ms_meet(s, k, fx_E, my_theta_g, xch, item.query);
            if (PROF) tc_meet += __builtin_readcyclecounter() - t_m0;
          }
        }

        if (PROF) tc_walk += __builtin_readcyclecounter() - t_win0;
        g = window_of_take((uint32_t)__builtin_amdgcn_readfirstlane((int)g_new));
        if (g < win_base || g >= win_base + part_wins) break;
      }
    }
    const uint64_t t_idle0 = PROF ? __builtin_readcyclecounter() : 0ull;
    while (ms_meet(s, k, fx_E, my_theta_g, xch, item.query)) {
    }
    const uint64_t t_epi0 = PROF ? __builtin_readcyclecounter() : 0ull;
    if (PROF && lane == 0) {
      atomicAdd((unsigned long long*)&s.prof[10], (unsigned long long)tc_meet);
      atomicAdd((unsigned long long*)&s.prof[11], (unsigned long long)(t_epi0 - t_idle0));
      atomicAdd((unsigned long long*)&s.prof[12], (unsigned long long)tc_part);
      atomicAdd((unsigned long long*)&s.prof[13], (unsigned long long)(tc_walk - tc_meet));
  #ifndef NRT_MS_COUNT_ROUNDS
      atomicMax((unsigned long long*)&s.prof[14], (unsigned long long)(t_idle0 - t_item0));
  #else
      atomicAdd((unsigned long long*)&s.prof[14], (unsigned long long)pc_half | ((unsigned long long)pc_half_rounds << 32));
      atomicAdd((unsigned long long*)&s.prof[11], (unsigned long long)pc_tas - (unsigned long long)(t_epi0 - t_idle0));
      atomicAdd((unsigned long long*)&s.prof[12], (unsigned long long)pc_dense - (unsigned long long)tc_part);
      atomicAdd((unsigned long long*)&s.prof[10], (unsigned long long)pc_sparse - (unsigned long long)tc_meet);
      atomicAdd((unsigned long long*)&s.prof[13], (unsigned long long)pc_steps - (unsigned long long)(tc_walk - tc_meet));
      atomicAdd((unsigned long long*)&s.prof[8], (unsigned long long)pc_crounds);
      atomicAdd((unsigned long long*)&s.prof[9], (unsigned long long)pc_cres);
      atomicAdd((unsigned long long*)&s.prof[15], (unsigned long long)pc_cinst);
  #endif
    }

    {
      const uint32_t c = s.cnt;
      __syncthreads();
      if (c > k) {
        uint64_t thr = 0;
        const uint32_t m = topk_compact<kMsThreads, kMsCandCap>(s.cand, c, k, &s.sc, &thr);
        if (tid == 0) s.cnt = m;
      }
    }
    if (lane == 0 && wave_hits) atomicAdd(&s.slot_hits[cur_slot], wave_hits);
  #ifdef NRT_MS_PHASE_CLOCKS
    if (PROF && lane == 0) {
  #pragma unroll
      for (int i = 0; i < 9; ++i) atomicAdd((unsigned long long*)&s.prof[i], (unsigned long long)ph[i]);
    }
    if (false) {
  #else
    if (PROF && lane == 0) {
      atomicAdd((unsigned long long*)&s.prof[0], (unsigned long long)pc_wins);
      atomicAdd((unsigned long long*)&s.prof[2], (unsigned long long)pc_chunks);
    }
    if (PROF) {
  #endif
      uint64_t v3 = pc_post, v4 = pc_surv, v6 = pc_look, v7 = pc_cand;
  #pragma unroll
      for (int dlt = 32; dlt > 0; dlt >>= 1) {
        v3 += __shfl_xor(v3, dlt, 64);
        v4 += __shfl_xor(v4, dlt, 64);
        v6 += __shfl_xor(v6, dlt, 64);
        v7 += __shfl_xor(v7, dlt, 64);
      }
      if (lane == 0) {
        atomicAdd((unsigned long long*)&s.prof[3], (unsigned long long)v3);
        atomicAdd((unsigned long long*)&s.prof[4], (unsigned long long)v4);
        atomicAdd((unsigned long long*)&s.prof[6], (unsigned long long)v6);
        atomicAdd((unsigned long long*)&s.prof[7], (unsigned long long)v7);
      }
    }
    __syncthreads();
    const uint32_t n_held = s.cnt;
    const ms_args_ptr ape = ms_fresh(launch);
    const __attribute__((address_space(4))) DHelp& hpe = ape->help;
    uint64_t* out = as_global(ape->item_keys) + (size_t)out_slot * ape->k_stride;
    if (tid == 0) {
      uint64_t th_end = s.theta;
      if (multi_item) {
        const uint64_t tg = (uint64_t)__hip_atomic_load(my_theta_g, __ATOMIC_RELAXED, __HIP_MEMORY_SCOPE_AGENT);
        if (tg > th_end) th_end = tg;
      }
      s.thr = th_end;
      s.cnt_valid = 0u;
    }
    __syncthreads();
    for (uint32_t i = tid; i < n_held; i += kMsThreads) {
      const uint64_t key = s.cand[i];
      if (key >= s.thr) out[atomicAdd(&s.cnt_valid, 1u)] = key;
    }
    __syncthreads();
    const uint32_t n = s.cnt_valid;
    if (tid == 0) {
      as_global(ape->item_counts)[out_slot] = n;
      if (helper)
        as_global(hpe.help_query)[out_slot - hpe.slot_base] = item.query + 1u;
      uint32_t hits = 0;
      for (int i = 0; i < kSliceSlots; ++i) {
        const uint32_t h = s.slot_hits[i];
        hits += h;
        if (h != 0u && q.gte_floor != 0xFFFFFFFFu) atomicAdd(as_global(ape->slice_sum) + q.slice_base + s.slot_slice[i], h);
      }
      const bool pruned = s.prune_on != 0u && (s.theta != 0ull || __hip_atomic_load(my_theta_g, __ATOMIC_RELAXED, __HIP_MEMORY_SCOPE_AGENT) != 0ull);
      as_global(ape->item_hits)[out_slot] = (uint64_t)hits + (pruned ? kHitsPrunedUnit : 0ull);
      if (PROF && ape->item_prof) {
  #ifndef NRT_MS_PHASE_CLOCKS
        s.prof[5] = hits;
        s.prof[1] = (s.prof[1] & 0xFFFull) | ((uint64_t)min(s.n_meet, 0xFFFu) << 12) | ((uint64_t)min(s.n_over, 0xFFFu) << 24) |
                    ((uint64_t)min(s.n_est & 0xFFFFu, 0xFFFu) << 36) | ((uint64_t)min(s.n_est >> 16, 0xFFFu) << 48);
  #endif
  #ifndef NRT_MS_COUNT_ROUNDS
        const uint64_t t_end = __builtin_readcyclecounter();
        s.prof[9] = t_end - t_item0;
        s.prof[15] = t_end - t_epi0;
  #endif
        for (int i = 0; i < 16; ++i) as_global(ape->item_prof)[(size_t)out_slot * 16 + i] = s.prof[i];
        if (hpe.walls) {
          unsigned long long* const wr = as_global(hpe.walls) + (size_t)out_slot * 8;
          wr[0] = wall0;
          wr[1] = wall_clock64();
          wr[2] = (unsigned long long)my_item | ((unsigned long long)item.flags << 32);
          wr[3] = s.prof[0];
          wr[4] = wall_entry;
          wr[5] = ((unsigned long long)((uint32_t)__builtin_amdgcn_s_getreg((31 << 11) | 20) & 15u) << 8) |
                  (unsigned long long)(((uint32_t)__builtin_amdgcn_s_getreg((31 << 11) | 4) >> 8) & 255u);
          wr[6] = (unsigned long long)round | ((unsigned long long)item.query << 32);
          wr[7] = blockIdx.x;
        }
      }
    }
    if (hpe.persistent == 0u) return;
    __syncthreads();
  }
}

__global__ __launch_bounds__(256)
void term_frontier_kernel(const uint32_t* __restrict__ fnorm, const uint64_t* __restrict__ t_start,
                          const uint32_t* __restrict__ t_count, const uint64_t* __restrict__ t_look,
                          const uint32_t* __restrict__ t_meta, const char* __restrict__ look_base, DTermAux* __restrict__ out) {
  __shared__ uint32_t mn[13];
  __shared__ uint32_t mf;
  const uint32_t t = blockIdx.x;
  if (threadIdx.x < 13) mn[threadIdx.x] = 0xFFu;
  if (threadIdx.x == 13) mf = 0u;
  __syncthreads();
  const uint64_t st = t_start[t];
  const uint32_t n = t_count[t];
  uint32_t lmn[13];
  uint32_t lmf = 0;
#pragma unroll
  for (int i = 0; i < 13; ++i) lmn[i] = 0xFFu;
  for (uint32_t p = threadIdx.x; p < n; p += 256u) {
    const uint32_t c = fnorm[st + p];
    if (c >> 31) {
      lmn[12] = min(lmn[12], c & 255u);
      lmf = max(lmf, (c >> 8) & 0x3FFFFFu);
    } else {
      const uint32_t f = (c >> 9) & 15u, nb = (c >> 2) & 127u;
#pragma unroll
      for (int i = 0; i < 12; ++i)
        if (f == (uint32_t)(i + 1)) lmn[i] = min(lmn[i], nb);
    }
  }
#pragma unroll
  for (int i = 0; i < 13; ++i)
    if (lmn[i] != 0xFFu) atomicMin(&mn[i], lmn[i]);
  if (lmf) atomicMax(&mf, lmf);
  __syncthreads();
  if (threadIdx.x == 0) {
    DTermAux a;
    const bool has = t_look[t] != ~0ull;
    a.look = has ? (const void*)(look_base + t_look[t]) : nullptr;
    for (int i = 0; i < 12; ++i) a.min_norm[i] = (uint8_t)mn[i];
    a.esc_min_norm = (uint8_t)mn[12];
    a.look_kind = has ? (uint8_t)(t_meta[t] & 255u) : (uint8_t)kLookNone;
    a.look_shift = has ? (uint8_t)((t_meta[t] >> 8) & 255u) : (uint8_t)0;
    a.pad = 0;
    a.esc_max_freq = mf;
    a.pad2 = 0;
    out[t] = a;
  }
}

__global__ __launch_bounds__(256)
void term_bits_kernel(const uint32_t* __restrict__ docids, const uint64_t* __restrict__ t_start, const uint32_t* __restrict__ t_count,
                      const uint64_t* __restrict__ t_look, const uint32_t* __restrict__ which, char* __restrict__ look_base) {
  const uint32_t t = which[blockIdx.y];
  const uint64_t st = t_start[t];
  const uint32_t n = t_count[t];
  uint32_t* const r = (uint32_t*)(look_base + t_look[t]);
  const uint32_t stride = gridDim.x * blockDim.x;
  for (uint32_t p = blockIdx.x * blockDim.x + threadIdx.x; p < n; p += stride) {
    const uint32_t d = docids[st + p];
    const uint32_t blk = d >> 5;
    atomicOr(&r[(size_t)blk * 2u], 1u << (d & 31u));
    if (p == 0u || (docids[st + p - 1u] >> 5) != blk) r[(size_t)blk * 2u + 1u] = p;
  }
}

__global__ __launch_bounds__(256)
void term_cells_kernel(const uint32_t* __restrict__ docids, const uint64_t* __restrict__ t_start, const uint32_t* __restrict__ t_count,
                       const uint64_t* __restrict__ t_look, const uint32_t* __restrict__ t_meta, const uint32_t* __restrict__ which,
                       uint32_t max_doc, char* __restrict__ look_base) {
  const uint32_t t = which[blockIdx.y];
  const uint32_t* const dd = docids + t_start[t];
// ... 90 lines not shown
```

nrtsearch_amd/csrc/runtime.cpp:

```cpp
#include "runtime_internal.h"

namespace nrtgpu {
namespace rt {
thread_local std::string g_last_error;
thread_local int64_t g_deadline_ns = 0;
thread_local nrtgpu_diagnostics g_diag{};
thread_local std::vector<int32_t> g_thread_slices;
int64_t monotonic_ns() {
  timespec ts;
  clock_gettime(CLOCK_MONOTONIC, &ts);
  return (int64_t)ts.tv_sec * 1000000000ll + (int64_t)ts.tv_nsec;
}

int fail(int code, const char* fmt, ...) {
  char buf[1024];
  va_list ap;
  va_start(ap, fmt);
  vsnprintf(buf, sizeof(buf), fmt, ap);
  va_end(ap);
  g_last_error = buf;
  return code;
}


// ... 205 lines not shown
    close(fd);
    return fail(NRTGPU_ERR_HIP, "ftruncate(%s, %zu) failed: %s", shm_name, bytes, strerror(errno));
  }
  void* p = mmap(nullptr, bytes, PROT_READ | PROT_WRITE, MAP_SHARED, fd, 0);
  close(fd);
  if (p == MAP_FAILED) return fail(NRTGPU_ERR_HIP, "mmap(%s) failed: %s", shm_name, strerror(errno));
  unsigned long long* t = (unsigned long long*)p;
  for (int sl = 0; sl < kExchangeSlots; ++sl)
    memset(t + ((size_t)sl * world + rank) * stride, 0, stride * 8);
  hipError_t e = hipHostRegister(p, bytes, hipHostRegisterMapped | hipHostRegisterPortable);
  void* dp = nullptr;
  if (e == hipSuccess) e = hipHostGetDevicePointer(&dp, p, 0);
  if (e != hipSuccess) {
    (void)munmap(p, bytes);
    return fail(NRTGPU_ERR_HIP, "mapping the exchange table into the GPU failed: %s", hipGetErrorString(e));
  }
  ctx->xch_host = p;
  ctx->xch_dev = (unsigned long long*)dp;
  ctx->xch_bytes = bytes;
  ctx->xch_world = world;
  ctx->xch_rank = rank;
  return NRTGPU_OK;
}

extern "C" void nrtgpu_destroy(nrtgpu_ctx* ctx) {
  if (!ctx) return;
  ctx->launcher.reset();
  nrtgpu_dist_close(ctx);
  nrtgpu_exchange_close(ctx);
  (void)hipSetDevice(ctx->device);
  for (auto& s : ctx->slots) {
    if (s->stream) (void)hipStreamSynchronize(s->stream);
    s->h_plan.release();
    s->d_plan.release();
    s->d_work.release();
    s->d_aux.release();
    s->h_aux.release();
    s->h_out.release();
    if (s->ev0) (void)hipEventDestroy(s->ev0);
    if (s->ev1) (void)hipEventDestroy(s->ev1);
    if (s->ev2) (void)hipEventDestroy(s->ev2);
    if (s->ev3) (void)hipEventDestroy(s->ev3);
    if (s->ev_turn) (void)hipEventDestroy(s->ev_turn);
    if (s->ev_wait) (void)hipEventDestroy(s->ev_wait);
    for (hipEvent_t e : s->round_ev) (void)hipEventDestroy(e);
    if (s->stream) (void)hipStreamDestroy(s->stream);
  }
  delete ctx;
}

extern "C" int nrtgpu_set_slicing(nrtgpu_ctx* ctx, int32_t slice_max_docs, int32_t slice_max_segments, int32_t virtual_shards) {
  if (!ctx || slice_max_docs < 0 || slice_max_segments <= 0 || virtual_shards <= 0) return fail(NRTGPU_ERR_INVALID_ARG, "bad slicing parameters");
  ctx->slice_max_docs = slice_max_docs;
  ctx->slice_max_segments = slice_max_segments;
  ctx->virtual_shards = virtual_shards;
  return NRTGPU_OK;
}

extern "C" int nrtgpu_set_thread_slices(const int32_t* slice_of_leaf, int32_t n_leaves) {
  if (n_leaves < 0 || (n_leaves > 0 && !slice_of_leaf)) return fail(NRTGPU_ERR_INVALID_ARG, "bad thread slices");
  for (int32_t i = 0; i < n_leaves; ++i)
    if (slice_of_leaf[i] < 0) return fail(NRTGPU_ERR_INVALID_ARG, "slice_of_leaf[%d] = %d: slice numbers are >= 0", i, slice_of_leaf[i]);
  g_thread_slices.assign(slice_of_leaf, slice_of_leaf + n_leaves);
  return NRTGPU_OK;
}

extern "C" int nrtgpu_get_stats(nrtgpu_ctx* ctx, nrtgpu_stats* out) {
  if (!ctx || !out) return fail(NRTGPU_ERR_INVALID_ARG, "NULL argument");
  std::lock_guard<std::mutex> lk(ctx->stats_mu);
  *out = ctx->stats;
  out->spec_queries = ctx->spec_queries.load(std::memory_order_relaxed);
  out->spec_reruns = ctx->spec_reruns.load(std::memory_order_relaxed);
  out->spec_disabled = ctx->spec_off.load(std::memory_order_relaxed);
  out->spec_scattered = ctx->spec_scattered.load(std::memory_order_relaxed);
  return NRTGPU_OK;
}
extern "C" void nrtgpu_reset_stats(nrtgpu_ctx* ctx) {
  if (!ctx) return;
  std::lock_guard<std::mutex> lk(ctx->stats_mu);
  ctx->stats = nrtgpu_stats{};
  for (double& p : ctx->prof) p = 0;
  for (double& p : ctx->ms_prof) p = 0;
  for (int64_t& p : ctx->ms_meetings) p = 0;
}
#ifdef NRTGPU_DEV
extern "C" int nrtgpu_get_scan_profile(nrtgpu_ctx* ctx, double* out16) {
  if (!ctx || !out16) return fail(NRTGPU_ERR_INVALID_ARG, "NULL argument");
  std::lock_guard<std::mutex> lk(ctx->stats_mu);
  for (int i = 0; i < 16; ++i) out16[i] = ctx->prof[i];
  return NRTGPU_OK;
}

extern "C" int nrtgpu_get_maxscore_profile(nrtgpu_ctx* ctx, double* out16) {
  if (!ctx || !out16) return fail(NRTGPU_ERR_INVALID_ARG, "NULL argument");
  std::lock_guard<std::mutex> lk(ctx->stats_mu);
  for (int i = 0; i < 16; ++i) out16[i] = ctx->ms_prof[i];
  return NRTGPU_OK;
}

extern "C" int64_t nrtgpu_get_maxscore_item_walls(nrtgpu_ctx* ctx, uint64_t* out, int64_t cap_slots, int64_t* n_items) {
  if (!ctx) return fail(NRTGPU_ERR_INVALID_ARG, "NULL argument");
  std::lock_guard<std::mutex> lk(ctx->stats_mu);
  const int64_t n = (int64_t)(ctx->last_walls.size() / 8);
  if (n_items) *n_items = ctx->last_walls_items;
  if (out)
    for (int64_t i = 0; i < std::min(n, cap_slots) * 8; ++i) out[i] = ctx->last_walls[(size_t)i];
  return n;
}
#endif

extern "C" int32_t nrtgpu_int_to_byte4(int32_t length) { return hostmath::int_to_byte4(length); }
extern "C" int32_t nrtgpu_byte4_to_int(int32_t b) { return hostmath::byte4_to_int(b); }
extern "C" float nrtgpu_bm25_idf(int64_t doc_count, int64_t doc_freq) { return hostmath::bm25_idf(doc_count, doc_freq); }
extern "C" float nrtgpu_bm25_avgdl(int64_t sttf, int64_t doc_count) { return hostmath::bm25_avgdl(sttf, doc_count); }
extern "C" void nrtgpu_bm25_norm_cache(float avgdl, float k1, float b, float* out256) { hostmath::bm25_norm_cache(avgdl, k1, b, out256); }

extern "C" int nrtgpu_fixed_point_scale(float weight, const float* norm_cache256, int32_t max_norm, int32_t* out_scale) {
  if (!norm_cache256 || !out_scale || max_norm < 0 || max_norm > 255) return fail(NRTGPU_ERR_INVALID_ARG, "bad fixed_point_scale arguments");
  return fixed_scale_of_term(weight, norm_cache256, (uint32_t)max_norm, out_scale) ? 1 : 0;
}

extern "C" int nrtgpu_blend(int32_t n_retrievers, const int32_t* const* docs, const float* const* scores, const int32_t* counts,
                            const float* boosts, int32_t mode, int32_t rank_constant, int32_t start_hit, int32_t top_hits,
                            nrtgpu_topdocs* out) {
  if (n_retrievers < 0 || (n_retrievers > 0 && (!docs || !counts)) || !out || top_hits < 0 || start_hit < 0 || (mode != 0 && mode != 1))
    return fail(NRTGPU_ERR_INVALID_ARG, "bad blend arguments");
  if (mode == 0 && rank_constant < 1) return fail(NRTGPU_ERR_INVALID_ARG, "k must be >= 1, got: %d", rank_constant);
  if (mode == 1 && n_retrievers > 0 && !scores) return fail(NRTGPU_ERR_INVALID_ARG, "score-order blend needs the retrievers' scores");
  for (int32_t r = 0; r < n_retrievers; ++r)
    if (counts[r] < 0 || (counts[r] > 0 && (!docs[r] || (mode == 1 && !scores[r])))) return fail(NRTGPU_ERR_INVALID_ARG, "bad retriever %d", r);
  std::vector<hostmath::BlendHit> page;
  const int64_t total = hostmath::blend_hits(n_retrievers, docs, scores, counts, boosts, rank_constant, mode == 0, start_hit, top_hits, &page);
  const int32_t cap = out->capacity > 0 ? out->capacity : top_hits;
  const int32_t m = std::min<int32_t>((int32_t)page.size(), cap);
  for (int32_t i = 0; i < m; ++i) {
    if (out->docs) out->docs[i] = page[(size_t)i].doc;
    if (out->scores) out->scores[i] = page[(size_t)i].score;
  }
  out->n_hits = m;
  out->total_hits = total;
  out->total_hits_is_lower_bound = 1;
  return NRTGPU_OK;
}

extern "C" int nrtgpu_plan_item_counts(int32_t n_queries, const int64_t* query_costs, int32_t target_items, int64_t* out_items) {
  if (n_queries < 0 || (n_queries > 0 && (!query_costs || !out_items)) || target_items <= 0)
    return fail(NRTGPU_ERR_INVALID_ARG, "bad plan_item_counts arguments");
  hostmath::plan_item_counts(query_costs, n_queries, target_items, (int64_t)1 << 17, out_items);
  return NRTGPU_OK;
}

extern "C" int32_t nrtgpu_slices(int32_t n_leaves, const int32_t* max_docs, const int32_t* num_docs, const int32_t* doc_bases,
                                 int32_t virtual_shards, int32_t slice_max_docs, int32_t slice_max_segments,
                                 int32_t* slice_of_leaf, int32_t* shard_of_leaf) {
  if (n_leaves < 0 || (n_leaves > 0 && (!max_docs || !slice_of_leaf))) return fail(NRTGPU_ERR_INVALID_ARG, "bad leaf arrays");
  std::vector<hostmath::LeafInfo> all((size_t)n_leaves);
  int32_t base = 0;
  for (int32_t i = 0; i < n_leaves; ++i) {
    all[(size_t)i] = {i, max_docs[i], num_docs ? num_docs[i] : max_docs[i], doc_bases ? doc_bases[i] : base};
    base += max_docs[i];
  }
  std::vector<std::vector<int32_t>> sl;
  std::vector<int32_t> shard;
  if (virtual_shards > 1) {
    sl = hostmath::slices_for_shards(all, virtual_shards, slice_max_docs, slice_max_segments, &shard);
  } else {
// ... 9 lines not shown
```

nrtsearch_amd/csrc/runtime_internal.h:

```cpp
#pragma once
#include <hip/hip_runtime.h>
#include <fcntl.h>
#include <stdarg.h>
#include <stdio.h>
#include <string.h>
#include <sys/mman.h>
#include <unistd.h>

#include <algorithm>
#include <atomic>
#include <cerrno>
#include <climits>
#include <cmath>
#include <chrono>
#include <condition_variable>
#include <deque>
#include <functional>
#include <map>
#include <memory>
#include <mutex>
#include <optional>
#include <shared_mutex>
#include <string>
#include <thread>
// ... 375 lines not shown
  hipEvent_t ev0 = nullptr, ev1 = nullptr, ev2 = nullptr, ev3 = nullptr;
  hipEvent_t ev_turn = nullptr;
  hipEvent_t ev_wait = nullptr;
  PinBuf h_plan;
  DevBuf d_plan;
  DevBuf d_work;
  DevBuf d_aux;
  PinBuf h_aux;
  PinBuf h_out;
  std::vector<hipEvent_t> round_ev;
  bool busy = false;
};

inline void forget_foreign_hip_error() { (void)hipGetLastError(); }

inline hipError_t wait_for_stream(bool blocking, hipStream_t st, hipEvent_t blocking_event) {
  if (!blocking) return hipStreamSynchronize(st);
  const hipError_t e = hipEventRecord(blocking_event, st);
  return e != hipSuccess ? e : hipEventSynchronize(blocking_event);
}

}
}

namespace nrtgpu {
namespace rt {
struct LeafSetCache;

class WorkPool {
 public:
  explicit WorkPool(int helpers);
  ~WorkPool();
  void run(int n, const std::function<void(int)>& fn);
  int helpers() const { return (int)threads_.size(); }

 private:
  struct Job {
    const std::function<void(int)>* fn;
    int n;
    std::atomic<int> next{0}, done{0};
  };
  void loop();
  std::vector<std::thread> threads_;
  std::mutex mu_;
  std::condition_variable cv_;
  std::vector<std::shared_ptr<Job>> jobs_;
  bool stop_ = false;
};
}
}

struct nrtgpu_dist;

struct Launcher {
  std::thread th;
  std::mutex mu;
  std::condition_variable cv;
  std::deque<std::function<void()>> q;
  bool stop = false;
  explicit Launcher(int device);
  ~Launcher();
  void push(std::function<void()> f);
};

struct nrtgpu_ctx {
  nrtgpu_config cfg{};
  nrtgpu_dist* dist = nullptr;
  int device = 0;
  int n_cus = 0;
  std::mutex mu;
  std::condition_variable cv;
  std::vector<std::unique_ptr<Slot>> slots;
  hipEvent_t last_turn = nullptr;
  hipEvent_t last_knn_turn = nullptr;
  std::mutex gpu_mu;
  std::mutex stats_mu;
  nrtgpu_stats stats{};
  std::atomic<int32_t> knn_gather_permille{0};
  std::atomic<int> knn_sketch_skip[4] = {};
  double prof[16] = {0};
  std::vector<uint64_t> last_walls;
  int64_t last_walls_items = 0;
  double ms_prof[16] = {0};
  int64_t ms_meetings[5] = {0};
  nrtgpu::rt::Coalescer co, kco, rco, bkco, brco;
  int32_t co_linger_us = 150;
  std::atomic<int64_t> spec_queries{0}, spec_reruns{0};
  std::atomic<int> spec_off{0};
  std::atomic<int> spec_scattered{0};
  std::atomic<uint64_t> spec_epoch{1};
  std::atomic<int> spec_z16{5 * 16};
  std::atomic<int64_t> shard_docs{0}, index_docs{0};
  std::atomic<int64_t> live_segments{0};
  std::atomic<int32_t> slice_max_docs{250000}, slice_max_segments{5}, virtual_shards{1};
  std::unique_ptr<nrtgpu::rt::WorkPool> pool;
  std::mutex launcher_mu;
  std::unique_ptr<Launcher> launcher;
  std::mutex lsc_mu;
  std::vector<std::shared_ptr<nrtgpu::rt::LeafSetCache>> leaf_sets;
  void* xch_host = nullptr;
  unsigned long long* xch_dev = nullptr;
  size_t xch_bytes = 0;
  int32_t xch_world = 0, xch_rank = 0;
};

namespace nrtgpu {
namespace rt {

struct Carver {
  size_t off = 0;
  size_t take(size_t bytes) {
    const size_t o = off;
    off += (bytes + 255) & ~(size_t)255;
    return o;
  }
};

struct TermLeaves {
  const DTerm* d_table = nullptr;
  std::vector<uint32_t> count;
  int64_t total = 0;
  uint32_t max_norm = 0;
};
struct LeafSetCache {
  std::vector<uint64_t> uids;
  struct Key {
    int32_t field;
    int64_t hash;
    bool operator==(const Key& o) const { return field == o.field && hash == o.hash; }
  };
  struct KeyHash {
    size_t operator()(const Key& k) const { return (size_t)(((uint64_t)k.hash ^ ((uint64_t)(uint32_t)k.field << 40)) * 0x9E3779B97F4A7C15ull >> 7); }
  };
  static const int kStripes = 64;
  static const size_t kMaxEntries = 1 << 20;
  struct Stripe {
    std::shared_mutex mu;
    std::unordered_map<Key, std::shared_ptr<const TermLeaves>, KeyHash> map;
  };
  Stripe stripes[kStripes];
  int device = 0;
  std::mutex arena_mu;
  std::vector<void*> chunks;
  size_t chunk_used = 0;
  static const size_t kChunkBytes = 1 << 20;
  static const size_t kMaxChunks = 256;
  bool full() {
    {
      std::lock_guard<std::mutex> lk(arena_mu);
      if (chunks.size() > kMaxChunks) return true;
    }
    return entries() > kMaxEntries;
  }
  void* alloc_tables(size_t stride, size_t want, size_t* got);
  ~LeafSetCache();
  uint64_t id = 0;
  std::atomic<int64_t> spec_queries{0}, spec_reruns{0};
  std::atomic<int64_t> spec_calls{0}, spec_calls_rerun{0};
  std::atomic<int> spec_scattered{0};
  std::atomic<int> spec_off{0};
  std::atomic<uint64_t> spec_epoch{0};
  const TermLeaves* get(const nrtgpu_seg* const* segs, int32_t n_segs, int32_t field, int64_t hash);
  void get_many(const nrtgpu_seg* const* segs, int32_t n_segs, const Key* keys, size_t n, const TermLeaves** out);
  size_t entries();
};
std::shared_ptr<LeafSetCache> leaf_set_cache(nrtgpu_ctx* ctx, const nrtgpu_seg* const* segs, int32_t n_segs);
// ... 347 lines not shown
```

nrtsearch_amd/csrc/search.cpp:

```cpp
#include "runtime_internal.h"


static uint32_t spec_margin16(const nrtgpu_ctx* ctx) { return (uint32_t)std::max(ctx->spec_z16.load(std::memory_order_relaxed), 0); }
static void spec_sync_epoch(const nrtgpu_ctx* ctx, LeafSetCache* lsc) {
  const uint64_t e = ctx->spec_epoch.load(std::memory_order_relaxed);
  if (lsc->spec_epoch.exchange(e, std::memory_order_relaxed) != e) {
    lsc->spec_queries.store(0, std::memory_order_relaxed);
    lsc->spec_reruns.store(0, std::memory_order_relaxed);
    lsc->spec_calls.store(0, std::memory_order_relaxed);
    lsc->spec_calls_rerun.store(0, std::memory_order_relaxed);
    lsc->spec_scattered.store(0, std::memory_order_relaxed);
    lsc->spec_off.store(0, std::memory_order_relaxed);
  }
}
static bool speculating(nrtgpu_ctx* ctx, const nrtgpu_seg* const* segs, int32_t n_segs) {
  if (!ctx || spec_margin16(ctx) == 0u || !segs || n_segs <= 0) return false;
  for (int32_t i = 0; i < n_segs; ++i)
    if (!segs[i]) return false;
  std::shared_ptr<LeafSetCache> lsc = leaf_set_cache(ctx, segs, n_segs);
  spec_sync_epoch(ctx, lsc.get());
  return lsc->spec_off.load(std::memory_order_relaxed) == 0;
}
static void note_speculation_of(nrtgpu_ctx* ctx, LeafSetCache* lsc, int64_t n_queries, int64_t n_rerun) {
  spec_sync_epoch(ctx, lsc);
// ... 50 lines not shown
  bool allow_spec = false;
  int32_t spec_world = 1;
  uint64_t* ext_guess = nullptr;
  bool follow_up = false;
};

static size_t ms_helpers(const nrtgpu_ctx* ctx, const HostPlan& hp) {
  static const int env_helpers = (int)dev_env_int("NRTGPU_MS_HELPERS", -1);
  return hp.n_ms_items == 0 ? 0 : (size_t)(env_helpers >= 0 ? env_helpers : 4 * std::max(ctx->n_cus, 1));
}

struct SearchLayout : PlanLayout {
  size_t n_items, n_help, n_slots;
  bool use_xch, walk_rows, spec, profile;
  uint32_t spec_z16;
  int ablation;
  size_t quant, lower, xch, q_wins, ms_args, plan_bytes;
  size_t rows, ssum, qprune, hwin, hcnt, ht0, hhead, hnext, hoff, hqueue, hused, hstart, spec_g;
  size_t zero_bytes, prof, walls;
  SearchLayout(const nrtgpu_ctx* ctx, const HostPlan& hp, int32_t n_queries, uint32_t k_stride_out, const SearchOpts& o, size_t n_help_)
      : PlanLayout(hp, hp.items.size() + n_help_, (size_t)n_queries, k_stride_out), n_items(hp.items.size()), n_help(n_help_), n_slots(n_items + n_help_) {
    quant = plan.take(hp.list_idx.size() * 8);
    lower = plan.take(o.ext_hits ? hp.q_lower.size() * 8 : 0);
    use_xch = o.epoch >= 0 && ctx->xch_dev != nullptr;
    xch = plan.take(use_xch ? sizeof(DExchange) : 0);
    q_wins = plan.take(hp.q_wins.size() * 4);
    ms_args = plan.take(sizeof(MsArgs));
    plan_bytes = plan.off;
    walk_rows = hp.n_ms_items != 0 && dev_env_int("NRTGPU_MS_WALK_ROWS", 1) != 0;
    rows = work.take(walk_rows ? (size_t)hp.n_dterms * sizeof(DWalkRow) : 0);
    ssum = work.take((size_t)n_queries * hp.n_slices * 4), qprune = work.take((size_t)n_queries * 4);
    hwin = work.take(hp.n_ms_items * 4), hcnt = work.take(hp.n_ms_items * 4), ht0 = work.take(hp.n_ms_items * 8);
    hhead = work.take((size_t)n_queries * 4), hnext = work.take(n_help * 4), hoff = work.take(4);
    hqueue = work.take(4), hused = work.take(4), hstart = work.take(8);
    spec_z16 = spec_margin16(ctx);
    spec = o.allow_spec && spec_z16 != 0u && hp.n_ms_items != 0 && !use_xch && hp.lsc && hp.lsc->spec_off.load(std::memory_order_relaxed) == 0;
    spec_g = work.take(spec ? (size_t)n_queries * 8 : 0);
    zero_bytes = work.off - ssum;
    const int flag_variant = (ctx->cfg.flags >> 8) & 15;
    ablation = hp.clause_counting ? 8 : ((hp.masked && flag_variant == 0 && !(ctx->cfg.flags & NRTGPU_FLAG_NO_MASK_VARIANT)) ? 9 : flag_variant);
    profile = flag_variant == 7;
    prof = work.take((ablation == 7 || profile) ? n_slots * 128 : 0);
    walls = work.take(profile ? n_slots * 64 : 0);
  }
};

static MsArgs ms_launch_record(const nrtgpu_ctx* ctx, const HostPlan& hp, const SearchLayout& L, const char* db, char* wb, bool small) {
  DHelp help{};
  help.win_next = (uint32_t*)(wb + L.hwin);
  help.help_cnt = (uint32_t*)(wb + L.hcnt);
  help.item_t0 = (unsigned long long*)(wb + L.ht0);
  help.help_head = (uint32_t*)(wb + L.hhead);
  help.help_query = (uint32_t*)(wb + L.hnext);
  help.help_off = (uint32_t*)(wb + L.hoff);
  help.item_next = (uint32_t*)(wb + L.hqueue);
  help.help_used = (uint32_t*)(wb + L.hused);
  help.t_start = (unsigned long long*)(wb + L.hstart);
  {
    static const int env_help_alpha = (int)dev_env_int("NRTGPU_MS_HELP_ALPHA", 24);
    uint64_t wins = 0;
    for (size_t i = 0; i < hp.n_ms_items; ++i) wins += hp.items[i].flags >> 8;
    help.total_wins = (uint32_t)std::min<uint64_t>(wins, 0xFFFFFFFFull);
    help.alpha16 = (uint32_t)std::max(env_help_alpha, 0);
    static const int env_spare = (int)dev_env_int("NRTGPU_MS_SPARE_CUS", 8);
    help.n_cus = (uint32_t)std::max(ctx->n_cus - std::max(env_spare, 0), 1);
    if (small) help.n_cus = (uint32_t)std::max(env_spare, 1);
    help.persistent = ms_persistent() ? 1u : 0u;
  }
  help.n_own = (uint32_t)hp.n_ms_items;
  help.n_help = (uint32_t)L.n_help;
  help.slot_base = (uint32_t)L.n_items;
  static const int env_help_min = (int)dev_env_int("NRTGPU_MS_HELP_MIN", 16);
  static const bool env_help_greedy = dev_env_int("NRTGPU_MS_HELP_GREEDY", 0) != 0;
  help.min_rem = (uint32_t)std::min(std::max(env_help_min, 1), 0xFFFF) | (env_help_greedy ? 1u << 16 : 0u);
  help.walls = L.profile ? (unsigned long long*)(wb + L.walls) : nullptr;
  help.spec_g = L.spec ? (unsigned long long*)(wb + L.spec_g) : nullptr;
  help.spec_z16 = L.spec ? L.spec_z16 : 0u;
  {
    const int env_first = (int)dev_env_int("NRTGPU_MS_SPEC_FIRST", 2 * kMsWaves);
    const int env_grow = (int)dev_env_int("NRTGPU_MS_SPEC_GROW", 32);
    const bool env_meet = dev_env_int("NRTGPU_MS_SPEC_MEET", 0) != 0;
    const bool env_half = dev_env_int("NRTGPU_MS_HALF_GROUPS", 1) != 0;
    const bool env_keep_live = dev_env_int("NRTGPU_MS_KEEP_LIVE", 1) != 0;
    help.spec_sched = (uint32_t)std::min(std::max(env_first, 1), 255) | ((uint32_t)std::min(std::max(env_grow, 17), 255) << 8) | (env_meet ? 1u << 16 : 0u) |
                      (env_half ? 0u : 1u << 17) | (env_keep_live ? 0u : 1u << 18);
  }
  MsArgs ms_args{};
  ms_args.items = (const DItem*)(db + L.items);
  ms_args.parts = (const DPart*)(db + L.parts);
  ms_args.terms = (const DTerm*)(wb + L.terms);
  ms_args.queries = (const DQuery*)(db + L.queries);
  ms_args.caches = (const float*)(db + L.caches);
  ms_args.theta_g = (unsigned long long*)(db + L.theta);
  ms_args.slice_sum = (uint32_t*)(wb + L.ssum);
  ms_args.q_prune = (uint32_t*)(wb + L.qprune);
  ms_args.xch = L.use_xch ? (const DExchange*)(db + L.xch) : nullptr;
  ms_args.item_keys = (uint64_t*)(wb + L.item_keys);
  ms_args.item_counts = (uint32_t*)(wb + L.item_counts);
  ms_args.item_hits = (uint64_t*)(wb + L.item_hits);
  ms_args.item_prof = L.profile ? (uint64_t*)(wb + L.prof) : nullptr;
  ms_args.q_wins = (const uint32_t*)(db + L.q_wins);
  ms_args.rows = L.walk_rows ? (const DWalkRow*)(wb + L.rows) : nullptr;
  {
    const long forced = dev_env_int("NRTGPU_MS_SCATTER", -1);
    ms_args.scatter = forced >= 0 ? (forced != 0 ? 1u : 0u) : ((L.spec && hp.lsc->spec_scattered.load(std::memory_order_relaxed) != 0) ? 1u : 0u);
  }
  ms_args.k_stride = hp.k_stride;
  ms_args.help = help;
  return ms_args;
}

static int enqueue_search(nrtgpu_ctx* ctx, Slot* slot, const HostPlan& hp, int32_t n_queries, uint32_t k_stride_out, const SearchOpts& o,
                          DeviceRun* run, std::unique_lock<std::mutex>& gpu) {
  forget_foreign_hip_error();
  static const bool follow_up_on = dev_env_int("NRTGPU_FOLLOW_UP", 1) != 0;
  const bool small = o.follow_up && follow_up_on && hp.n_ms_items != 0 && hp.n_ms_items == hp.items.size() && ms_persistent();
  const SearchLayout L(ctx, hp, n_queries, k_stride_out, o, ms_helpers(ctx, hp));
  const size_t n_items = L.n_items, n_help = L.n_help, n_ms = hp.n_ms_items;
  if (int rc = slot->h_plan.reserve(L.plan_bytes)) return rc;
  if (int rc = slot->d_plan.reserve(L.plan_bytes)) return rc;
  if (int rc = slot->d_work.reserve(L.work.off)) return rc;
  char* hb = (char*)slot->h_plan.p;
  char* db = (char*)slot->d_plan.p;
  char* wb = (char*)slot->d_work.p;
  L.fill(hb, hp);
  PlanLayout::put(hb, L.q_wins, hp.q_wins.data(), hp.q_wins.size() * 4);
  if (o.spec_world > 1) {
    uint64_t num = (uint64_t)o.spec_world, den = 1;
    const int64_t sd = ctx->shard_docs.load(std::memory_order_relaxed), id = ctx->index_docs.load(std::memory_order_relaxed);
    if (sd > 0 && id >= sd) {
      num = (uint64_t)id;
      den = (uint64_t)sd;
    }
    uint32_t* qw = (uint32_t*)(hb + L.q_wins);
    for (size_t i = 0; i < hp.q_wins.size(); ++i) qw[i] = (uint32_t)std::min<uint64_t>(((uint64_t)qw[i] * num + den - 1) / den, 0xFFFFFFFFull);
  }
  memset(hb + L.quant, 0, hp.list_idx.size() * 8);
  if (o.ext_hits) memcpy(hb + L.lower, hp.q_lower.data(), hp.q_lower.size() * 8);
  if (L.use_xch) {
    DExchange x{};
    const size_t stride = (size_t)ctx->cfg.max_batch;
    x.slot = ctx->xch_dev + (size_t)(o.epoch % kExchangeSlots) * (size_t)ctx->xch_world * stride;
    x.world = (uint32_t)ctx->xch_world;
    x.rank = (uint32_t)ctx->xch_rank;
    x.stride = (uint32_t)stride;
    x.tag = (uint32_t)(o.epoch + 1);
    if (x.tag == 0) x.tag = 1;
    memcpy(hb + L.xch, &x, sizeof(x));
  }
  L.put_expand_head(hb, db, L.walk_rows ? (DWalkRow*)(wb + L.rows) : nullptr);
  const MsArgs ms_args = ms_launch_record(ctx, hp, L, db, wb, small);
  const DHelp& help = ms_args.help;
  memcpy(hb + L.ms_args, &ms_args, sizeof(ms_args));
  const bool profile = L.profile, use_xch = L.use_xch;
  const int ablation = L.ablation;

  hipStream_t st = slot->stream;
  HIP_TRY(hipMemcpyAsync(db, hb, L.plan_bytes, hipMemcpyHostToDevice, st));
  HIP_TRY(hipMemsetAsync(wb + L.ssum, 0, L.zero_bytes, st));
  const bool timing = ctx->cfg.collect_timing != 0;
  launch_expand_terms(st, (const DQExpand*)(db + L.qexpand), (const DQTerm*)(db + L.qterms), (const uint32_t*)(db + L.qs_begin),
                      (uint32_t)n_queries, hp.n_leaves, (DTerm*)(wb + L.terms));
  gpu.lock();
  static const bool overlap_scorers = dev_env_int("NRTGPU_OVERLAP_SCORERS", 0) != 0;
  if (ctx->last_turn && !overlap_scorers && !small) HIP_TRY(hipStreamWaitEvent(st, ctx->last_turn, 0));
  if (ctx->last_knn_turn) HIP_TRY(hipStreamWaitEvent(st, ctx->last_knn_turn, 0));
  if (timing) HIP_TRY(hipEventRecord(slot->ev3, st));
  if (profile && n_help) HIP_TRY(hipMemsetAsync(wb + L.prof + n_items * 128, 0, n_help * 128, st));
// ... 105 lines not shown
  for (int si = 0; si < n_segs; ++si)
    if (!segs[si]) return fail(NRTGPU_ERR_INVALID_ARG, "segment %d is NULL", si);
  return NRTGPU_OK;
}

static int search_batch_impl(nrtgpu_ctx* ctx, const nrtgpu_seg* const* segs, const int32_t* doc_bases,
                             int32_t n_segs, const nrtgpu_bm25_query* queries, int32_t n_queries,
                             nrtgpu_topdocs* out, std::vector<int32_t>* rerun, bool content_held = false, const uint64_t* seeds = nullptr,
                             bool follow_up = false) {
  if (!ctx || !queries || !out || (n_segs > 0 && !segs)) return fail(NRTGPU_ERR_INVALID_ARG, "NULL argument");
  if (int rc = check_batch_size(ctx, n_queries, n_segs)) return rc;
  NRT_CHECK_DEADLINE("before the search was planned");
  const double t0 = now_ms();
  if (int rc = enter_search(ctx, segs, n_segs)) return rc;
  HostPlan hp;
  std::optional<SegReadLocks> content;
  if (!content_held) content.emplace(segs, n_segs);
  if (int rc = build_plan(ctx, segs, doc_bases, n_segs, queries, n_queries, hp, 1)) return rc;
  if (seeds)
    for (int qi = 0; qi < n_queries; ++qi) hp.theta_init[(size_t)qi] = std::max(hp.theta_init[(size_t)qi], seeds[qi]);
  const double plan_ms = now_ms() - t0;

  Slot* slot = nullptr;
  acquire_slot(ctx, &slot);
  SlotGuard guard{ctx, slot};
  const double queue_ms = now_ms() - t0 - plan_ms;
  NRT_CHECK_DEADLINE("while the search waited for a workspace");
  DeviceRun run;
  const size_t kb = (size_t)n_queries * hp.k_stride * 8, cb = (size_t)n_queries * 4, hb = (size_t)n_queries * 8;
  Carver oc;
  const size_t o_k = oc.take(kb), o_c = oc.take(cb), o_h = oc.take(hb);
  if (int rc = slot->h_out.reserve(oc.off)) return rc;
  char* ho = (char*)slot->h_out.p;
  static const bool call_trace = dev_env_int("NRTGPU_PLAN_TRACE", 0) != 0;
  const double tc0 = call_trace ? now_ms() : 0.0;
  {
    std::unique_lock<std::mutex> gpu(ctx->gpu_mu, std::defer_lock);
    SearchOpts o;
    o.allow_spec = rerun != nullptr;
    o.follow_up = follow_up;
    if (int rc = enqueue_search(ctx, slot, hp, n_queries, hp.k_stride, o, &run, gpu)) return rc;
  }
  const double tc1 = call_trace ? now_ms() : 0.0;
  if ((const char*)run.out_counts - (const char*)run.out_keys == (ptrdiff_t)(o_c - o_k) && (const char*)run.out_hits - (const char*)run.out_keys == (ptrdiff_t)(o_h - o_k)) {
    HIP_TRY(hipMemcpyAsync(ho + o_k, run.out_keys, (o_h - o_k) + hb, hipMemcpyDeviceToHost, slot->stream));
  } else {
    HIP_TRY(hipMemcpyAsync(ho + o_k, run.out_keys, kb, hipMemcpyDeviceToHost, slot->stream));
    HIP_TRY(hipMemcpyAsync(ho + o_c, run.out_counts, cb, hipMemcpyDeviceToHost, slot->stream));
    HIP_TRY(hipMemcpyAsync(ho + o_h, run.out_hits, hb, hipMemcpyDeviceToHost, slot->stream));
  }
  HIP_TRY(wait_for_stream((ctx->cfg.flags & NRTGPU_FLAG_BLOCKING_WAIT) != 0, slot->stream, slot->ev_wait));
  const double tc2 = call_trace ? now_ms() : 0.0;
  const uint64_t* keys = (const uint64_t*)(ho + o_k);
  const uint32_t* cnts = (const uint32_t*)(ho + o_c);
  const uint64_t* hits = (const uint64_t*)(ho + o_h);
  {
    const int n_chunks = n_queries >= 256 ? std::min(8, ctx->pool->helpers() + 1) : 1;
    ctx->pool->run(n_chunks, [&](int c) {
      const int q0 = (int)((int64_t)n_queries * c / n_chunks), q1 = (int)((int64_t)n_queries * (c + 1) / n_chunks);
      for (int qi = q0; qi < q1; ++qi)
        unpack_topdocs(keys + (size_t)qi * hp.k_stride, cnts[qi], hits[qi] & ~kHitsSpecInvalid, queries[qi].k, hp.q_lower[(size_t)qi], cnts[qi], &out[qi]);
    });
  }
  if (rerun)
    for (int qi = 0; qi < n_queries; ++qi)
      if (hits[qi] & kHitsSpecInvalid) rerun->push_back(qi);
  if (call_trace)
    fprintf(stderr, "[nrtgpu call] %d queries: plan %.3f ms, upload + kernels %.3f, results to host %.3f, unpack %.3f\n", n_queries, plan_ms,
            tc1 - tc0, tc2 - tc1, now_ms() - tc2);
  if (run.prof && run.n_items) {
    std::vector<uint64_t> hp_prof(run.n_slots * 16);
    HIP_TRY(hipMemcpy(hp_prof.data(), run.prof, hp_prof.size() * 8, hipMemcpyDeviceToHost));
    std::lock_guard<std::mutex> lk(ctx->stats_mu);
    for (size_t i = 0; i < run.n_slots; ++i)
      if (i < run.n_ms_items || i >= run.n_items) {
#ifndef NRT_MS_PHASE_CLOCKS
        const uint64_t packed = hp_prof[i * 16 + 1];
        hp_prof[i * 16 + 1] = packed & 0xFFFull;
        ctx->ms_meetings[0] += (int64_t)((packed >> 12) & 0xFFFull);
        ctx->ms_meetings[1] += (int64_t)((packed >> 24) & 0xFFFull);
        ctx->ms_meetings[2] += (int64_t)(packed & 0xFFFull);
        ctx->ms_meetings[3] += (int64_t)((packed >> 36) & 0xFFFull);
        ctx->ms_meetings[4] += (int64_t)((packed >> 48) & 0xFFFull);
#endif
        for (int j = 0; j < 16; ++j) ctx->ms_prof[j] += (double)hp_prof[i * 16 + j];
      } else {
        for (int j = 0; j < 16; ++j) ctx->prof[j] += (double)hp_prof[i * 16 + j];
      }
    if (run.walls) {
      std::vector<uint64_t> w(run.n_slots * 8);
      (void)hipMemcpy(w.data(), run.walls, w.size() * 8, hipMemcpyDeviceToHost);
      ctx->last_walls.swap(w);
      ctx->last_walls_items = (int64_t)run.n_ms_items;
    }
  }
  account(ctx, slot, hp, n_queries, plan_ms, t0, queue_ms);
  return NRTGPU_OK;
}

typedef std::function<void(const std::vector<int32_t>&)> AfterFirst;
template <class Pass>
static int two_pass_search(nrtgpu_ctx* ctx, const nrtgpu_seg* const* segs, int32_t n_segs, const nrtgpu_bm25_query* queries, int32_t n_queries,
                           nrtgpu_topdocs* out, const AfterFirst* after_first, const Pass& pass) {
  if (!speculating(ctx, segs, n_segs)) return pass(queries, n_queries, out, nullptr, nullptr);
  if (ctx && segs)
    for (int si = 0; si < n_segs; ++si)
      if (!segs[si]) return fail(NRTGPU_ERR_INVALID_ARG, "segment %d is NULL", si);
  std::vector<int32_t> rerun;
  SegReadLocks content(segs, n_segs);
  if (int rc = pass(queries, n_queries, out, &rerun, nullptr)) return rc;
  note_speculation(ctx, segs, n_segs, n_queries, (int64_t)rerun.size());
  if (rerun.empty()) return NRTGPU_OK;
  if (after_first) (*after_first)(rerun);
  std::vector<nrtgpu_bm25_query> rq(rerun.size());
  std::vector<nrtgpu_topdocs> ro(rerun.size());
  for (size_t i = 0; i < rerun.size(); ++i) {
    rq[i] = queries[rerun[i]];
    ro[i] = out[rerun[i]];
  }
  DeadlineScope no_deadline(true);
  if (int rc = pass(rq.data(), (int32_t)rq.size(), ro.data(), nullptr, rerun.data())) return rc;
  for (size_t i = 0; i < rerun.size(); ++i) out[rerun[i]] = ro[i];
  return NRTGPU_OK;
}

static int search_batch_spec(nrtgpu_ctx* ctx, const nrtgpu_seg* const* segs, const int32_t* doc_bases, int32_t n_segs,
                             const nrtgpu_bm25_query* queries, int32_t n_queries, nrtgpu_topdocs* out, const AfterFirst* after_first) {
  nrtgpu_diagnostics first{};
  bool second = false;
  const int rc = two_pass_search(ctx, segs, n_segs, queries, n_queries, out, after_first,
                                 [&](const nrtgpu_bm25_query* q, int32_t n, nrtgpu_topdocs* o, std::vector<int32_t>* rerun, const int32_t* idx) {
    if (!idx) {
      const int rc1 = search_batch_impl(ctx, segs, doc_bases, n_segs, q, n, o, rerun, rerun != nullptr);
      if (rerun) first = g_diag;
      return rc1;
    }
    std::vector<uint64_t> seeds((size_t)n, 0ull);
    static const bool seed_reruns = dev_env_int("NRTGPU_SEED_RERUNS", 1) != 0;
    for (int32_t i = 0; i < n; ++i) {
      const int32_t k = q[i].k;
      if (seed_reruns && k > 0 && o[i].n_hits >= k && o[i].docs && o[i].scores && (o[i].capacity <= 0 || o[i].capacity >= k)) {
        const uint64_t kth = pack_key(o[i].scores[k - 1], (uint32_t)o[i].docs[k - 1]);
        seeds[(size_t)i] = kth > 0 ? kth - 1 : 0ull;
      }
    }
    second = true;
    return search_batch_impl(ctx, segs, doc_bases, n_segs, q, n, o, nullptr, true, seeds.data(), n <= 32);
  });
  if (rc != 0 || !second) return rc;
  nrtgpu_diagnostics d = g_diag;
  d.total_ms += first.total_ms;
  d.plan_ms += first.plan_ms;
  d.queue_ms += first.queue_ms;
  d.device_ms += first.device_ms;
  d.postings += first.postings;
  d.queries = first.queries;
  d.items_maxscore += first.items_maxscore;
  d.items_scan += first.items_scan;
  g_diag = d;
  return NRTGPU_OK;
}

extern "C" int nrtgpu_search_bm25_batch(nrtgpu_ctx* ctx, const nrtgpu_seg* const* segs, const int32_t* doc_bases,
                                        int32_t n_segs, const nrtgpu_bm25_query* queries, int32_t n_queries,
                                        nrtgpu_topdocs* out) {
  return search_batch_spec(ctx, segs, doc_bases, n_segs, queries, n_queries, out, nullptr);
// ... 625 lines not shown
```

Baseline: 570,600.

## Add presence-bitmap candidate generation for windows whose tail clauses are dense bitsets

For MaxScore windows where the trailing clauses are stored as dense presence bitmaps, the kernel now ORs together the ANDs of the minimal clause subsets whose summed upper bound can reach the threshold. This produces candidate docs directly from the bitmaps instead of walking postings of those clauses. Candidates are compacted four per lane through LDS and scored with a new walk_units specialization that looks up every clause. The aim is to avoid iterating dense posting lists, at the cost of added register pressure, extra kernel code and LDS traffic. It also adds debug counters and environment knobs, and the path is enabled by default.

```diff
diff --git a/include/nrtgpu_dev.h b/include/nrtgpu_dev.h
--- a/include/nrtgpu_dev.h
+++ b/include/nrtgpu_dev.h
@@ -23,6 +23,7 @@
 int  nrtgpu_get_maxscore_profile(nrtgpu_ctx* ctx, double* out16);
 int  nrtgpu_debug_maxscore_meetings(nrtgpu_ctx* ctx, int64_t* out4);
 int  nrtgpu_debug_maxscore_meeting_guesses(nrtgpu_ctx* ctx, int64_t* out1);
+int  nrtgpu_debug_maxscore_presence(nrtgpu_ctx* ctx, int64_t* out3);
 int  nrtgpu_debug_wave_kth(const uint64_t* keys, int32_t n, int32_t r, uint64_t* out);
 int64_t nrtgpu_debug_walk_rows(nrtgpu_ctx* ctx, const nrtgpu_seg* const* segs, const int32_t* doc_bases, int32_t n_segs,
                                const nrtgpu_bm25_query* queries, int32_t n_queries, int32_t* out_begin, int32_t* out_n,
diff --git a/nrtsearch_amd/_lib.py b/nrtsearch_amd/_lib.py
--- a/nrtsearch_amd/_lib.py
+++ b/nrtsearch_amd/_lib.py
@@ -65,7 +65,7 @@
     "nrtgpu_debug_spec_counters", "nrtgpu_get_scan_profile", "nrtgpu_get_maxscore_profile", "nrtgpu_get_maxscore_item_walls",
     "nrtgpu_debug_dist_inject", "nrtgpu_debug_term_lookup", "nrtgpu_debug_knn_bounds", "nrtgpu_debug_knn_unpack",
     "nrtgpu_debug_maxscore_meetings", "nrtgpu_debug_wave_kth", "nrtgpu_debug_walk_rows", "nrtgpu_debug_walk_value",
-    "nrtgpu_debug_maxscore_meeting_guesses",
+    "nrtgpu_debug_maxscore_meeting_guesses", "nrtgpu_debug_maxscore_presence",
 ]
 DEV_LIB_PATH = os.path.join(_HERE, "libnrtgpu_dev.so")
 
@@ -297,6 +297,8 @@
         L.nrtgpu_debug_wave_kth.argtypes = [vp, i32, i32, vp]
     if hasattr(L, "nrtgpu_debug_maxscore_meeting_guesses"):
         L.nrtgpu_debug_maxscore_meeting_guesses.argtypes = [vp, vp]
+    if hasattr(L, "nrtgpu_debug_maxscore_presence"):
+        L.nrtgpu_debug_maxscore_presence.argtypes = [vp, vp]
     if hasattr(L, "nrtgpu_debug_walk_rows"):
         L.nrtgpu_debug_walk_rows.argtypes = [vp, vp, vp, i32, vp, i32, vp, vp, vp, i64]
         L.nrtgpu_debug_walk_rows.restype = C.c_int64
diff --git a/nrtsearch_amd/api.py b/nrtsearch_amd/api.py
--- a/nrtsearch_amd/api.py
+++ b/nrtsearch_amd/api.py
@@ -366,6 +366,11 @@
         _lib.check(_lib.load().nrtgpu_debug_maxscore_meeting_guesses(self._h, g.ctypes.data))
         res["meeting_guesses"] = int(g[0])
         return res
+
+    def maxscore_presence(self) -> dict:
+        out = np.zeros(3, dtype=np.int64)
+        _lib.check(_lib.load().nrtgpu_debug_maxscore_presence(self._h, out.ctypes.data))
+        return dict(zip(["windows", "candidate_docs", "windows_with_streamed_record_clauses"], (int(x) for x in out)))
 
     @staticmethod
     def set_thread_deadline(seconds_from_now: Optional[float]) -> None:
diff --git a/nrtsearch_amd/csrc/devtools.cpp b/nrtsearch_amd/csrc/devtools.cpp
--- a/nrtsearch_amd/csrc/devtools.cpp
+++ b/nrtsearch_amd/csrc/devtools.cpp
@@ -101,6 +101,13 @@
   return NRTGPU_OK;
 }
 
+extern "C" int nrtgpu_debug_maxscore_presence(nrtgpu_ctx* ctx, int64_t* out3) {
+  if (!ctx || !out3) return fail(NRTGPU_ERR_INVALID_ARG, "NULL argument");
+  std::lock_guard<std::mutex> lk(ctx->stats_mu);
+  for (int i = 0; i < 3; ++i) out3[i] = ctx->ms_presence[i];
+  return NRTGPU_OK;
+}
+
 extern "C" int nrtgpu_debug_maxscore_meeting_guesses(nrtgpu_ctx* ctx, int64_t* out1) {
   if (!ctx || !out1) return fail(NRTGPU_ERR_INVALID_ARG, "NULL argument");
   std::lock_guard<std::mutex> lk(ctx->stats_mu);
diff --git a/nrtsearch_amd/csrc/maxscore.hip b/nrtsearch_amd/csrc/maxscore.hip
--- a/nrtsearch_amd/csrc/maxscore.hip
+++ b/nrtsearch_amd/csrc/maxscore.hip
@@ -256,11 +256,101 @@
   return wbase + wave_total <= (uint32_t)kMsCandCap;
 }
 
+constexpr uint32_t kMsNoPresence = 0xFFFFFFFFu;
+__device__ __noinline__ uint32_t ms_presence_window(__attribute__((address_space(3))) MsSmem* sp, uint32_t wave, uint32_t n_terms, uint32_t my_flags,
+                                                    uint64_t my_suf, uint64_t thr_w, uint32_t my_count, uint32_t win_tiles) {
+  MsSmem& s = *(MsSmem*)sp;
+  const uint32_t lane = threadIdx.x & 63u;
+#ifdef NRTGPU_DEV
+  const uint32_t knobs = (uint32_t)__builtin_amdgcn_readfirstlane((int)s.spec_meet);
+  if ((knobs & 8u) != 0u) return kMsNoPresence;
+  const bool scan_all = (knobs & 16u) != 0u;
+  const uint32_t pres_min = (knobs >> 5) != 0u ? (knobs >> 5) * 32u : kMsPresenceMin;
+#else
+  constexpr bool scan_all = false;
+  constexpr uint32_t pres_min = kMsPresenceMin;
+#endif
+  const uint32_t rec = (uint32_t)__builtin_amdgcn_ballot_w64(lane < n_terms && ((my_flags >> 24) & 7u) == kLookBits);
+  if (rec == 0u) return kMsNoPresence;
+  const uint32_t r0 = (uint32_t)__builtin_ctz(rec);
+  if (rec != ((uint32_t)((1ull << n_terms) - 1ull) & ~((1u << r0) - 1u)) || n_terms - r0 > (uint32_t)kMsPresenceClauses) return kMsNoPresence;
+  const uint64_t my_ub = lane < n_terms ? my_suf - s.wc[wave][lane].u_after : 0ull;
+  const uint32_t alone = scan_all ? 0u : (uint32_t)__builtin_amdgcn_ballot_w64(lane >= r0 && lane < n_terms && my_ub >= thr_w);
+  const uint32_t r1 = alone != 0u ? 32u - (uint32_t)__builtin_clz(alone) : r0;
+  if (!scan_all && r1 + 3u > n_terms) return kMsNoPresence;
+  const bool mine = lane >= r1 && lane < n_terms && my_suf >= thr_w;
+  const uint32_t dense = (uint32_t)__builtin_amdgcn_readlane((int)scan32_dpp(mine ? my_count : 0u), kMsMaxTerms - 1);
+  if (dense == 0u || dense < max(pres_min * win_tiles / (uint32_t)kMsWinTiles, 1u)) return kMsNoPresence;
+  return r0 | (r1 << 8);
+}
+
+constexpr int kScanSteps = 8;
+static_assert(kMsWinWords % (64 * kScanSteps) == 0 && kMsWinWords / 64 <= 32, "a window's scan: whole passes, one bit per 64 words");
+__device__ __noinline__ uint32_t ms_presence_scan(__attribute__((address_space(3))) MsSmem* sp, uint32_t which, uint64_t min_sets, uint32_t doc_lo, uint32_t doc_span,
+                                              uint32_t w0) {
+  MsSmem& s = *(MsSmem*)sp;
+  const uint32_t lane = threadIdx.x & 63u, wave = threadIdx.x >> 6;
+  const uint32_t r0 = which & 255u, nr = (which >> 8) & 255u, n_out = (which >> 16) & 255u;
+  const bool use_seen = (which >> 24) != 0u;
+  uint32_t* const seen = &s.seen[wave][0];
+  const uint64_t sets = uniform_u64(min_sets);
+  if ((w0 & (64u * (uint32_t)kScanSteps - 1u)) != 0u) return seen[w0 + lane];
+  uint32_t first = 0;
+  {
+    uint32_t bits[kScanSteps][kMsPresenceClauses];
+#pragma unroll
+    for (int i = 0; i < kMsPresenceClauses; ++i) {
+      if ((uint32_t)i < nr) {
+        const gu32_ptr recs = (gu32_ptr)uniform_u64(s.wc[wave][r0 + (uint32_t)i].look) + (size_t)(doc_lo >> 5) * 2u;
+#pragma unroll
+        for (int t = 0; t < kScanSteps; ++t) {
+          const uint32_t word = w0 + 64u * (uint32_t)t + lane;
+          bits[t][i] = recs[word * 32u < doc_span ? word * 2u : 0u];
+        }
+      } else {
+#pragma unroll
+        for (int t = 0; t < kScanSteps; ++t) bits[t][i] = 0u;
+      }
+    }
+    uint32_t m[kScanSteps];
+#pragma unroll
+    for (int t = 0; t < kScanSteps; ++t) m[t] = 0u;
+    for (uint64_t left = sets; left != 0ull; left &= left - 1ull) {
+      const uint32_t set = (uint32_t)__builtin_ctzll(left);
+#pragma unroll
+      for (int t = 0; t < kScanSteps; ++t) {
+        uint32_t x = 0xFFFFFFFFu;
+#pragma unroll
+        for (int i = 0; i < kMsPresenceClauses; ++i)
+          if ((set >> i) & 1u) x &= bits[t][i];
+        m[t] |= x;
+      }
+    }
+#pragma unroll
+    for (int t = 0; t < kScanSteps; ++t) {
+      const uint32_t word = w0 + 64u * (uint32_t)t + lane;
+#pragma unroll
+      for (int i = 0; i < kMsPresenceClauses; ++i)
+        if ((uint32_t)i < n_out) m[t] &= ~bits[t][i];
+      if (use_seen) m[t] &= ~seen[word];
+      const uint32_t rem = word * 32u < doc_span ? doc_span - word * 32u : 0u;
+      if (rem < 32u) m[t] &= (1u << rem) - 1u;
+      if (t != 0) seen[word] = m[t];
+      else first = m[t];
+    }
+  }
+  wave_lds_phase();
+  return first;
+}
+
 template <bool PROF, bool PACKED, int SHAPES>
 __global__ __launch_bounds__(kMsThreads)
 void bm25_maxscore_kernel(const MsArgs* __restrict__ launch) {
   constexpr bool TWO = SHAPES == 2;
   constexpr bool kMsHalfBody = kSl == 8;
+  constexpr bool kPresence = SHAPES == 0 && !PACKED;
+  constexpr uint32_t kNoPresence = kMsNoPresence;
+  constexpr int kPresSlots = 4;
   __shared__ MsSmem s;
   const uint32_t tid = threadIdx.x;
   const uint32_t wave = tid >> 6, lane = tid & 63u;
@@ -410,7 +500,7 @@
       s.spec_slot = spec ? as_global(hp.spec_g) + item.query : nullptr;
       s.spec_at = spec ? max(hp.spec_sched & 255u, 1u) : 0u;
       s.spec_grow16 = max((hp.spec_sched >> 8) & 255u, 17u);
-      s.spec_meet = (hp.spec_sched >> 16) & 7u;
+      s.spec_meet = hp.spec_sched >> 16;
       for (int i = 0; i < kSliceSlots; ++i) s.slot_hits[i] = s.slot_slice[i] = 0u;
       for (int i = 0; i < 16; ++i) s.prof[i] = 0;
     }
@@ -443,6 +533,8 @@
     uint32_t wave_hits = 0;
     uint32_t cur_slot = 0;
     uint64_t pc_post = 0, pc_surv = 0, pc_look = 0, pc_cand = 0, pc_chunks = 0, pc_wins = 0;
+    uint64_t pc_pres_wins = 0, pc_pres_docs = 0;
+    uint64_t pc_pres_split = 0;
   #ifdef NRT_MS_PHASE_CLOCKS
     uint64_t ph[9] = {0, 0, 0, 0, 0, 0, 0, 0, 0}, ph_t = 0;
   #endif
@@ -646,11 +738,17 @@
           for (int j = 0; j < kMsWinWords / 64 / 4; ++j) *(u32x4*)&seen[(lane + 64u * (uint32_t)j) * 4u] = u32x4{0u, 0u, 0u, 0u};
         }
         uint32_t ng = 0;
+        uint32_t pres = kNoPresence;
         {
-          const uint64_t thr_w = __hip_atomic_load(&s.prune_on, __ATOMIC_RELAXED, __HIP_MEMORY_SCOPE_WORKGROUP) ? loosen(max(s.thr, thr_other)) : 0ull;
+          const bool prune_w = __hip_atomic_load(&s.prune_on, __ATOMIC_RELAXED, __HIP_MEMORY_SCOPE_WORKGROUP) != 0u;
+          const uint64_t thr_w = prune_w ? loosen(max(s.thr, thr_other)) : 0ull;
           const uint64_t pb = my_start + my_lo, pe = my_start + my_hi;
+          if constexpr (kPresence) {
+            if (prune_w) pres = ms_presence_window((__attribute__((address_space(3))) MsSmem*)&s, wave, n_terms, my_flags, my_suf, thr_w,
+                                                   (uint32_t)min(pe - pb, (uint64_t)0xFFFFFFu), win_tiles);
+          }
           if (lane < n_terms) {
-            if (my_suf >= thr_w && pe > pb && (!SHAPES || msm <= 1u || lane + msm <= n_terms) && (!TWO || lane <= first_req)) ng = (uint32_t)((pe - (pb & ~3ull) + (uint64_t)(kSl - 1)) / (uint64_t)kSl);
+            if (my_suf >= thr_w && pe > pb && (!SHAPES || msm <= 1u || lane + msm <= n_terms) && (!TWO || lane <= first_req) && lane < (pres >> 8)) ng = (uint32_t)((pe - (pb & ~3ull) + (uint64_t)(kSl - 1)) / (uint64_t)kSl);
             *(u32x4*)&wcl[lane].begin = u32x4{(uint32_t)pb, (uint32_t)(pb >> 32), (uint32_t)(pe - pb), 0u};
           }
         }
@@ -669,9 +767,11 @@
         if (PROF) ph_t = t_win0;
   #endif
         NRT_PH_MARK(0);
-        auto walk_units = [&](auto ns_c, auto half_c, const uint32_t v0) __attribute__((always_inline)) -> bool {
+        auto walk_units = [&](auto ns_c, auto half_c, auto pres_c, const uint32_t v0, const uint32_t (&pd)[kPresSlots], const uint32_t pd_mask) __attribute__((always_inline)) -> bool {
           constexpr int NS = decltype(ns_c)::value;
           constexpr bool HALF = decltype(half_c)::value;
+          constexpr bool PRES = decltype(pres_c)::value;
+          static_assert(!PRES || (NS == kPresSlots && !HALF && kPresence), "a presence window's candidates: four per lane, plain sums");
           static_assert(!HALF || (NS == 4 && kSl == 8), "the half body: four of a unit's eight postings per lane");
           const uint32_t n_lanes = HALF ? 2u * (n_groups - v0) : min(n_groups - v0, 64u);
           const uint32_t v = HALF ? v0 + (lane >> 1) : v0 + lane;
@@ -682,11 +782,25 @@
             c += (v >= pre[i]) ? 1u : 0u;
             before = (v >= pre[i]) ? pre[i] : before;
           }
+          if constexpr (PRES) c = v0;
           const uint32_t c_first = (uint32_t)__builtin_amdgcn_readfirstlane((int)c);
           const uint64_t theta = max(s.theta, theta_other), thr = loosen(max(s.thr, thr_other));
           const bool pruning = __hip_atomic_load(&s.prune_on, __ATOMIC_RELAXED, __HIP_MEMORY_SCOPE_WORKGROUP) != 0u;
           const uint64_t thr_p = pruning ? thr : 0ull;
-          if (readlane_u64(my_suf, c_first) < thr_p) return false;
+          if (readlane_u64(my_suf, PRES ? c_first + 1u : c_first) < thr_p) return false;
+          uint32_t d[NS];
+          uint64_t run[NS];
+          uint32_t alive = 0;
+          uint64_t sec[TWO ? NS : 1];
+          if constexpr (PRES) {
+  #pragma unroll
+            for (int j = 0; j < NS; ++j) {
+              d[j] = pd[j];
+              run[j] = 0ull;
+            }
+            alive = pd_mask;
+            if (PROF) pc_pres_docs += (uint64_t)__popc(alive);
+          } else {
           if (PROF) pc_chunks += 1;
           const uint32_t rec = wcl_addr + c * (uint32_t)sizeof(WClause);
           const u32x4 r0 = *(const u32x4*)lds_ptr(rec), r1 = *(const u32x4*)lds_ptr(rec + 16u), r2 = *(const u32x4*)lds_ptr(rec + 32u);
@@ -696,7 +810,7 @@
           const uint32_t flags = r2[2];
           const uint32_t q0 = (v - before) * (uint32_t)kSl + (HALF ? (lane & 1u) * 4u : 0u);
           const uint64_t mine0 = (p_begin & ~3ull) + (uint64_t)q0;
-          uint32_t d[NS], cd[NS];
+          uint32_t cd[NS];
   #pragma unroll
           for (int j = 0; j < NS; ++j) d[j] = cd[j] = 0u;
           if (act) {
@@ -765,8 +879,6 @@
               }
             }
           }
-          uint64_t run[NS];
-          uint32_t alive = 0;
           {
             const uint32_t mult = 1u << ((flags >> 4) & 15u);
             uint32_t need_v = 1u;
@@ -788,7 +900,6 @@
                 if ((use_max ? max(run[j], u_after) : run[j] + u_after) < thr_p) alive &= ~(1u << j);
             }
           }
-          uint64_t sec[TWO ? NS : 1];
           if (TWO) {
             if ((req_mask & ((1u << c) - 1u)) != 0u) alive = 0u;
             const bool mine_counts = sec_mode == kMsSecTieBreaker || (sec_mode == kMsSecReqOpt && ((req_mask >> c) & 1u) == 0u);
@@ -821,12 +932,13 @@
             }
           }
           NRT_PH_MARK(3);
+          }
           uint32_t ccnt = 0x11111111u;
 
           for (uint32_t j2 = c_first + 1u; j2 < n_terms; ++j2) {
             if (!__any(alive != 0u)) break;
             const uint64_t S_j = readlane_u64(my_suf, j2);
-            uint32_t am = c < j2 ? alive : 0u;
+            uint32_t am = PRES || c < j2 ? alive : 0u;
             {
               const uint64_t short_of = S_j < thr_p ? (use_max ? thr_p : thr_p - S_j) : 0ull;
               uint32_t kill = 0;
@@ -855,7 +967,7 @@
   #ifdef NRT_MS_COUNT_ROUNDS
             if (PROF) { if (kind2 == kLookBits) pc_dense += 1; else pc_sparse += 1; }
   #endif
-            if (kind2 == kLookBits) {
+            if (PRES || kind2 == kLookBits) {
               const gvec2_ptr recs = (gvec2_ptr)look2;
               u32x2 r[NS];
   #pragma unroll
@@ -1044,13 +1156,14 @@
           NRT_PH_MARK(8);
           return true;
         };
+        const uint32_t no_docs[kPresSlots] = {0u, 0u, 0u, 0u};
+        bool more = true;
         for (uint32_t v0 = 0; v0 < n_groups; v0 += 64u) {
-          bool more;
           if (kMsHalfBody && n_groups - v0 <= 32u && half_on) {
   #ifdef NRT_MS_COUNT_ROUNDS
             const uint64_t chunks0 = pc_chunks, look0 = pc_dense + pc_sparse;
   #endif
-            if constexpr (kMsHalfBody) more = walk_units(std::integral_constant<int, 4>{}, std::true_type{}, v0);
+            if constexpr (kMsHalfBody) more = walk_units(std::integral_constant<int, 4>{}, std::true_type{}, std::false_type{}, v0, no_docs, 0u);
             else more = false;
   #ifdef NRT_MS_COUNT_ROUNDS
             if (PROF) {
@@ -1059,13 +1172,81 @@
             }
   #endif
           } else {
-            more = walk_units(std::integral_constant<int, kSl>{}, std::false_type{}, v0);
+            more = walk_units(std::integral_constant<int, kSl>{}, std::false_type{}, std::false_type{}, v0, no_docs, 0u);
           }
           if (!more) break;
           if (__hip_atomic_load(&s.rz_flag, __ATOMIC_RELAXED, __HIP_MEMORY_SCOPE_WORKGROUP)) {
             const uint64_t t_m0 = PROF ? __builtin_readcyclecounter() : 0ull;
             (void)ms_meet(s, k, fx_E, my_theta_g, xch, item.query);
             if (PROF) tc_meet += __builtin_readcyclecounter() - t_m0;
+          }
+        }
+
+        if constexpr (kPresence) {
+          if (pres != kNoPresence && more) {
+            const uint32_t r0 = pres & 255u, r1 = pres >> 8, nr = n_terms - r0;
+            uint64_t sub = 0;
+            for (uint32_t i = 0; i < nr; ++i) {
+              const uint64_t ub = readlane_u64(my_suf, r0 + i) - (r0 + i + 1u < n_terms ? readlane_u64(my_suf, r0 + i + 1u) : 0ull);
+              if ((lane >> i) & 1u) sub += ub;
+            }
+            const uint64_t thr_s = max(s.thr, thr_other);
+            const uint64_t wins = __builtin_amdgcn_ballot_w64(lane < (1u << nr) && (lane & ((1u << (r1 - r0)) - 1u)) == 0u && sub >= thr_s);
+            bool minimal = ((wins >> lane) & 1ull) != 0ull;
+            for (uint32_t i = 0; i < nr; ++i)
+              if (((lane >> i) & 1u) && ((wins >> (lane & ~(1u << i))) & 1ull)) minimal = false;
+            const uint64_t min_sets = __builtin_amdgcn_ballot_w64(minimal);
+            if (PROF) {
+              pc_pres_wins += 1;
+              if (r1 > r0) pc_pres_split += 1;
+            }
+            uint32_t pd[kPresSlots] = {0u, 0u, 0u, 0u};
+            uint32_t pd_mask = 0, waiting = 0, m = 0, stage = 0, w0 = 0;
+            bool done = min_sets == 0ull;
+
+            while (!done) {
+              const uint64_t has = __builtin_amdgcn_ballot_w64(m != 0u);
+              if (has != 0ull) {
+                const uint32_t before = __builtin_amdgcn_mbcnt_hi((uint32_t)(has >> 32), __builtin_amdgcn_mbcnt_lo((uint32_t)has, 0u));
+                const uint32_t room = 64u * (uint32_t)kPresSlots - waiting;
+                const uint32_t n_new = min((uint32_t)__popcll(has), room);
+                if (m != 0u && before < room) {
+                  seen[stage + ((waiting + before) & 63u)] = doc_lo + (stage + lane) * 32u + (uint32_t)__builtin_ctz(m);
+                  m &= m - 1u;
+                }
+                wave_lds_phase();
+                const uint32_t got = seen[stage + lane];
+                const uint32_t turn = (lane - waiting) & 63u;
+                if (turn < n_new) {
+                  const uint32_t slot = (waiting + turn) >> 6;
+  #pragma unroll
+                  for (int j = 0; j < kPresSlots; ++j)
+                    if (slot == (uint32_t)j) pd[j] = got;
+                  pd_mask |= 1u << slot;
+                }
+                wave_lds_phase();
+                waiting += n_new;
+              } else if (w0 * 32u < doc_span) {
+                stage = w0;
+                w0 += 64u;
+                m = ms_presence_scan((__attribute__((address_space(3))) MsSmem*)&s, r0 | (nr << 8) | ((r1 - r0) << 16) | (r1 != 0u ? 1u << 24 : 0u), min_sets, doc_lo, doc_span, stage);
+                wave_lds_phase();
+                continue;
+              } else {
+                done = true;
+              }
+              if (waiting == 64u * (uint32_t)kPresSlots || (done && waiting != 0u)) {
+                more = walk_units(std::integral_constant<int, kPresSlots>{}, std::false_type{}, std::true_type{}, r1 - 1u, pd, pd_mask);
+                pd_mask = 0u;
+                waiting = 0u;
+                if (!more) break;
+                if (__hip_atomic_load(&s.rz_flag, __ATOMIC_RELAXED, __HIP_MEMORY_SCOPE_WORKGROUP)) {
+                  const uint64_t t_m0 = PROF ? __builtin_readcyclecounter() : 0ull;
+                  (void)ms_meet(s, k, fx_E, my_theta_g, xch, item.query);
+                  if (PROF) tc_meet += __builtin_readcyclecounter() - t_m0;
+                }
+              }
+            }
           }
         }
 
@@ -1115,24 +1296,26 @@
     if (false) {
   #else
     if (PROF && lane == 0) {
-      atomicAdd((unsigned long long*)&s.prof[0], (unsigned long long)pc_wins);
+      atomicAdd((unsigned long long*)&s.prof[0], (unsigned long long)pc_wins | ((unsigned long long)pc_pres_wins << 32) | ((unsigned long long)pc_pres_split << 48));
       atomicAdd((unsigned long long*)&s.prof[2], (unsigned long long)pc_chunks);
     }
     if (PROF) {
   #endif
-      uint64_t v3 = pc_post, v4 = pc_surv, v6 = pc_look, v7 = pc_cand;
+      uint64_t v3 = pc_post, v4 = pc_surv, v6 = pc_look, v7 = pc_cand, v2 = pc_pres_docs;
   #pragma unroll
       for (int dlt = 32; dlt > 0; dlt >>= 1) {
         v3 += __shfl_xor(v3, dlt, 64);
         v4 += __shfl_xor(v4, dlt, 64);
         v6 += __shfl_xor(v6, dlt, 64);
         v7 += __shfl_xor(v7, dlt, 64);
+        v2 += __shfl_xor(v2, dlt, 64);
       }
       if (lane == 0) {
         atomicAdd((unsigned long long*)&s.prof[3], (unsigned long long)v3);
         atomicAdd((unsigned long long*)&s.prof[4], (unsigned long long)v4);
         atomicAdd((unsigned long long*)&s.prof[6], (unsigned long long)v6);
         atomicAdd((unsigned long long*)&s.prof[7], (unsigned long long)v7);
+        atomicAdd((unsigned long long*)&s.prof[2], (unsigned long long)v2 << 32);
       }
     }
     __syncthreads();
@@ -1185,7 +1368,7 @@
           wr[0] = wall0;
           wr[1] = wall_clock64();
           wr[2] = (unsigned long long)my_item | ((unsigned long long)item.flags << 32);
-          wr[3] = s.prof[0];
+          wr[3] = (uint32_t)s.prof[0];
           wr[4] = wall_entry;
           wr[5] = ((unsigned long long)((uint32_t)__builtin_amdgcn_s_getreg((31 << 11) | 20) & 15u) << 8) |
                   (unsigned long long)(((uint32_t)__builtin_amdgcn_s_getreg((31 << 11) | 4) >> 8) & 255u);
diff --git a/nrtsearch_amd/csrc/runtime.cpp b/nrtsearch_amd/csrc/runtime.cpp
--- a/nrtsearch_amd/csrc/runtime.cpp
+++ b/nrtsearch_amd/csrc/runtime.cpp
@@ -311,6 +311,7 @@
   for (double& p : ctx->prof) p = 0;
   for (double& p : ctx->ms_prof) p = 0;
   for (int64_t& p : ctx->ms_meetings) p = 0;
+  for (int64_t& p : ctx->ms_presence) p = 0;
 }
 #ifdef NRTGPU_DEV
 extern "C" int nrtgpu_get_scan_profile(nrtgpu_ctx* ctx, double* out16) {
diff --git a/nrtsearch_amd/csrc/runtime_internal.h b/nrtsearch_amd/csrc/runtime_internal.h
--- a/nrtsearch_amd/csrc/runtime_internal.h
+++ b/nrtsearch_amd/csrc/runtime_internal.h
@@ -481,6 +481,7 @@
   std::vector<uint64_t> last_walls;
   int64_t last_walls_items = 0;
   double ms_prof[16] = {0};
+  int64_t ms_presence[3] = {0};
   int64_t ms_meetings[5] = {0};
   nrtgpu::rt::Coalescer co, kco, rco, bkco, brco;
   int32_t co_linger_us = 150;
diff --git a/nrtsearch_amd/csrc/search.cpp b/nrtsearch_amd/csrc/search.cpp
--- a/nrtsearch_amd/csrc/search.cpp
+++ b/nrtsearch_amd/csrc/search.cpp
@@ -156,8 +156,12 @@
     const bool env_meet = dev_env_int("NRTGPU_MS_SPEC_MEET", 0) != 0;
     const bool env_half = dev_env_int("NRTGPU_MS_HALF_GROUPS", 1) != 0;
     const bool env_keep_live = dev_env_int("NRTGPU_MS_KEEP_LIVE", 1) != 0;
+    const bool env_presence_all = dev_env_int("NRTGPU_MS_PRESENCE_ALL", 0) != 0;
+    const bool env_presence = dev_env_int("NRTGPU_MS_PRESENCE", 1) != 0;
+    const long env_presence_min = dev_env_int("NRTGPU_MS_PRESENCE_MIN", 0);
+    const uint32_t presence_min32 = env_presence_min > 0 ? (uint32_t)std::min(std::max((env_presence_min + 31) / 32, 1L), 2047L) : 0u;
     help.spec_sched = (uint32_t)std::min(std::max(env_first, 1), 255) | ((uint32_t)std::min(std::max(env_grow, 17), 255) << 8) | (env_meet ? 1u << 16 : 0u) |
-                      (env_half ? 0u : 1u << 17) | (env_keep_live ? 0u : 1u << 18);
+                      (env_half ? 0u : 1u << 17) | (env_keep_live ? 0u : 1u << 18) | (env_presence ? 0u : 1u << 19) | (env_presence_all ? 1u << 20 : 0u) | (presence_min32 << 21);
   }
   MsArgs ms_args{};
   ms_args.items = (const DItem*)(db + L.items);
@@ -429,6 +433,11 @@
         ctx->ms_meetings[2] += (int64_t)(packed & 0xFFFull);
         ctx->ms_meetings[3] += (int64_t)((packed >> 36) & 0xFFFull);
         ctx->ms_meetings[4] += (int64_t)((packed >> 48) & 0xFFFull);
+        ctx->ms_presence[0] += (int64_t)((hp_prof[i * 16 + 0] >> 32) & 0xFFFFull);
+        ctx->ms_presence[2] += (int64_t)(hp_prof[i * 16 + 0] >> 48);
+        ctx->ms_presence[1] += (int64_t)(hp_prof[i * 16 + 2] >> 32);
+        hp_prof[i * 16 + 0] &= 0xFFFFFFFFull;
+        hp_prof[i * 16 + 2] &= 0xFFFFFFFFull;
 #endif
         for (int j = 0; j < 16; ++j) ctx->ms_prof[j] += (double)hp_prof[i * 16 + j];
       } else {
```

Result: no change. 577,000, median of 5 (+1.1%).
